# IntelRealSense/hand_tracking_samples

Hardware: AMD Instinct MI355X
Metric: synthetic depth frames/sec (CNN+solver), 64x64x1 input, 17-bone hand (higher is better)
Workload: dtype f32; 1 GPU; BASELINE configs[2]: 1024 independent 64x64 frames per GPU, CNN + decode + 5-step MultiStepSim + 3 FitPointCloud passes (GJK + PGS), 17 bones; frames_per_gpu=1024, parallelism=single GPU

## Files before the change

hand_tracking_samples_amd/csrc/ht_launch.hpp:

```cpp
#pragma once
#include "ht_device.hpp"

struct solve_args
{
	const float *rows_pre; const int *n_pre; int pre_stride;
	const float *rows_cloud; const int *n_cloud;
	const unsigned char *cloud_body;
	const float *contacts; const int *ncontacts;
	const float *ang_user; const int *n_ang_user; int ang_user_stride;
	const float *lin_tail; const int *n_lin_tail; int lin_tail_stride;
	const unsigned short *lin_tail_pos; const int *n_tail_groups;
	int no_model_rows;
	const float *analysis; const float *cams;
	const int *active_flag;
	float *state;
	float *scratch; int scratch_stride;
	int batch;
	int apply_angles; float drive_force; int ray_rows; int arm_cone; int zero_momenta; int steps_keyangles; float min_cray_prob;
	const float *sf_crays; int sf_ncray; int sf_select; float sf_spoint[3], sf_rbpoint[3]; const float *sf_refpose; int sf_hold;
	int *caps;
	int shared_gpu;
	const int *frame_order; int *cost_out;
	int two_body_levels;
	int force_build;
	float *out_poses; const int *out_npts; int *out_initializing; int out_min_point_num;
	int ang_extra_bound;
	float *exact_lin, *exact_ang;
	const float *tables;
	int dbg;
};

#define TB_WORDS 8928
struct prep_args
{
	const float *state; const float *analysis; const float *cams; const int *active_flag;
	float *scratch; int scratch_stride; int batch;
	const unsigned char *cloud_body; const int *n_cloud;
	const float *ch_planes; const int *ch_on;
	float *rows_pre; int *n_pre; float ch_maxforce;
	int apply_angles; float drive_force; int ray_rows; int arm_cone; int steps_keyangles; float min_cray_prob;
	int parts;
	float *tables;
	int dbg;
};
void ht_launch_solve_prep(const ht_model_dev &M, const ht_physics_dev &ph, const prep_args &a, int B, hipStream_t s);

struct cloud_records { float *scratch; int stride; unsigned char *body; float dt; };
void ht_launch_cloud_rows(const ht_model_dev &M, const float *state, const float4 *pts, const int *npts, const float *cams, const int *active_flag, int stride, int use_cam_origin, int mode,
                          const ht_params &par, float *rows, int *nrows, int B, hipStream_t s, float sf_ratio = 0.0f, float sf_wrist = 0.0f, const cloud_records *rec = nullptr);
struct ht_fit_after
{
	int mode;
	float reset_thr; int angles_only; int *flags, *nflags; int *list, *nlist; unsigned *nreset;
	float *hand; const float *other; const float *err_old; float *prev_err; int *initializing, *accepted; int nb, min_point_num, always_take_cnn; float accum_thr;
};
void ht_launch_fit_error(const ht_model_dev &M, const float *state, const float4 *pts, const int *npts, const uint16_t *depth, const float *cams, int w, int h, float scale, float *err, int B, hipStream_t s, const ht_fit_after *after = nullptr);
void ht_launch_chamber(const ht_model_dev &M, const float *state, const float4 *pts, const int *npts, int min_point_num, int enabled, float maxforce, float *rows, int *nch, int B, hipStream_t s,
                       const float *planes = nullptr, const int *planes_on = nullptr);
void ht_launch_chamber_planes(const ht_model_dev &M, const float4 *pts, const int *npts, int min_point_num, int enabled, float *planes, int *on, int B, hipStream_t s);
void ht_launch_contacts(const ht_model_dev &M, const float *state, float driftmax, float jiggle_sin, const int *active_flag, void *epa_ws, float *contacts, int *ncontacts, int B, hipStream_t s, bool beside_cloud_rows = false, int force_kernel = 0, int few_frames = 0,
                        const int *order = nullptr, int *work_out = nullptr);
int ht_contacts_frames_per_block(const ht_model_dev &M, int B);
#define HT_CONTACT_SLOTS 16
void ht_launch_order_by_points(const int *npts, int *order, int B, hipStream_t s);
void ht_launch_rank_desc(const int *work, int *order, int B, int stride, unsigned slots, int nslots, hipStream_t s);
void ht_launch_contact_order(const int *work, int *order, int B, int nfr, int stride, unsigned slots, int nslots, int epb, hipStream_t s);
size_t ht_contacts_workspace_bytes(int B);
void ht_launch_solve(const ht_model_dev &M, const ht_physics_dev &ph, const solve_args &a, int B, hipStream_t s);
void ht_launch_set_pose(float *state, const float *src, int nb, int n, int mode, hipStream_t s);
void ht_launch_get_state(const float *state, float *dst, int nb, int n, hipStream_t s);
void ht_launch_clear_flags(float *prev_err, int *initializing, int n, hipStream_t s);
void ht_launch_reset(const ht_model_dev &M, const ht_physics_dev &ph, float *state, const float4 *pts, const int *npts, const float *analysis, const float *cams, const int *list, const int *nlist,
                     int n_unibody, const ht_params &par, float *rows, int *nrows, float *scratch, int scratch_stride, int batch, int B, hipStream_t s, bool many_frames, int n_cu, bool exact = false);
void ht_launch_output(const ht_model_dev &M, const float *hand, const int *npts, int *initializing, int min_point_num, float *poses, int n, hipStream_t s, int raw = 0);
bool ht_segment_supported(int w, int h);
void ht_launch_segment(const uint16_t *depth, const float *cams, int w, int h, int entry_options, float wrange_hi, float diam, uint16_t *tiles, float *cams_out, int B, hipStream_t s);
void ht_launch_scale_state(float *state, int nb, int n, float s, hipStream_t st);
void ht_launch_train_step(float *w, float *W2p, const float *x, const float *target, float alpha, float *act, float *err, float *part, float *mse_out, hipStream_t s);
size_t ht_train_act_floats();
size_t ht_train_err_floats();
size_t ht_train_part_floats();
```

hand_tracking_samples_amd/csrc/ht_solver.hip:

```cpp
#include "ht_solve_shared.hpp"

template <int NGRP_, int NSUM_, int NANG_, int NIDX_, int AS_ = 2, int NCG_ = 0> struct lds_t
{
	static constexpr int NGRP = NGRP_, NSUM = NSUM_, NANG = NANG_, NIDX = NIDX_, MAXA2 = MAXA2_OF(AS_), NCG = NCG_;
	static constexpr int LIDLE = MAXG - 1;
	float pool[NGRP * LGRP] __attribute__((aligned(16)));
	float4 lin4[HT_MAXNB];
	float4 ang4[HT_MAXNB];
	float pos[HT_MAXNB][3], q[HT_MAXNB][4];
	float csum[NSUM];
	unsigned short cidx[NIDX > 0 ? NIDX : 2];
	float cg[NCG];
	int ccnt[HT_MAXNB], cstart[HT_MAXNB];
	signed char cextra[HT_MAXNB];
	union
	{
		unsigned lorder[MAXG];
		struct { unsigned short abody[128]; unsigned etmp[64]; } blk;
	};
	unsigned short lstart[MAXG + 2];
	unsigned aorder[MAXA2 + 1];
	unsigned short astart[MAXA2 + 2];
	int nlev_lin, nlev_ang, nray;
	union
	{
		struct
		{
			float jr[HT_MAXNJ][6];
			float ray[36][HT_ROW];
			int aprefix[HT_MAXNJ + 1], rprefix[HT_MAXNJ + 1];
			unsigned char rowj[MAXA2];
			unsigned char lrb[MAXG][2], arb[MAXA2][2];
			unsigned char gst[MAXA_RUNS + 1];
			float4 I4[HT_MAXNB][3];
		};
		float arec[(NANG + 4) * AROW] __attribute__((aligned(16)));
	};
};


template <int NS, class Order, class Start>
__device__ __forceinline__ int level_schedule(int n, int lane, const int (&b0)[2], const int (&b1)[2], Order put_order, Start put_start)
{
	auto rdl = [](int v, int l) -> int { return __builtin_amdgcn_readlane(v, l); };
	int last = 0, lev[2] = { 0, 0 };
	for (int g = 0; g < n; g++)
	{
		const int l = g & 63;
		const bool hi = NS > 1 && g >= 64;
		const int x0 = hi ? rdl(b0[1], l) : rdl(b0[0], l), x1 = hi ? rdl(b1[1], l) : rdl(b1[0], l);
		const int l0 = x0 != 255 ? rdl(last, x0 & 63) : 0, l1 = x1 != 255 ? rdl(last, x1 & 63) : 0;
		const int lv = (l0 > l1 ? l0 : l1) + 1;
		last = (lane == x0 || lane == x1) ? lv : last;
		lev[0] = (lane == l && !hi) ? lv : lev[0];
		if (NS > 1) lev[1] = (lane == l && hi) ? lv : lev[1];
	}
	int lower[2] = { 0, 0 }, before[2] = { 0, 0 };
	for (int h = 0; h < n; h++)
	{
		const int lh = (NS > 1 && h >= 64) ? rdl(lev[1], h & 63) : rdl(lev[0], h & 63);
#pragma unroll
		for (int s = 0; s < NS; s++) { lower[s] += lh < lev[s] ? 1 : 0; before[s] += (lh == lev[s] && h < lane + 64 * s) ? 1 : 0; }
	}
	int key[2], sb[2] = { 0, 0 };
#pragma unroll
	for (int s = 0; s < 2; s++) key[s] = (s < NS && lane + 64 * s < n) ? lev[s] * 2 + ((before[s] & 7) == 0 ? 1 : 0) : 0x7ffffffe;
	for (int h = 0; h < n; h++)
	{
		const int kh = (NS > 1 && h >= 64) ? rdl(key[1], h & 63) : rdl(key[0], h & 63);
#pragma unroll
		for (int s = 0; s < NS; s++) sb[s] += ((kh >> 1) < lev[s]) ? (kh & 1) : 0;
	}
	int steps = 0;
#pragma unroll
	for (int s = 0; s < NS; s++)
	{
		const int g = lane + 64 * s;
		const bool valid = g < n, first = valid && (before[s] & 7) == 0;
		const int pos = lower[s] + before[s];
		if (valid) put_order(pos, g, s);
		if (first) put_start(1 + sb[s] + (before[s] >> 3), pos);
		steps += __popcll(__ballot(first));
	}
	if (lane == 0) { put_start(steps + 1, n); put_start(steps + 2, n); }
	return steps;
}

#define EX_LIN HT_EX_LIN
template <int NGRP_, int NSUM_, int NANG_, int NIDX_, bool EXACT = false, int AS = 2, int NCG_ = 0>
__global__ __launch_bounds__(64, 2) void k_solve(ht_model_dev M, ht_physics_dev ph, solve_args a)
{
	__shared__ lds_t<NGRP_, NSUM_, NANG_, NIDX_, AS, NCG_> S;
	constexpr int ASLOTS = AS, MAXA2 = MAXA2_OF(AS), MAXA_LDS = MAXA_CAP_OF(AS);
	const int lane = threadIdx.x;
	const int b = a.frame_order ? a.frame_order[blockIdx.x] : (int)blockIdx.x;
	if (a.active_flag && !a.active_flag[b]) return;
	const long long t_cost = a.cost_out ? clock64() : 0;
	const long long t_entry = HT_DBG(a.dbg, 2048) ? clock64() : 0;
	const int nb = M.nb, nj = M.nj;
	float *st = a.state + (size_t)b * nb * HT_STATE_STRIDE;
	const float dt = ph.deltaT;
	const float *const T = a.tables ? a.tables + (size_t)b * TB_WORDS : nullptr;
	bool fast_pose = false, fast_chain = false;
	int t_na = 0, t_npre = 0, t_total = 0, t_e0 = 0, t_nblk = 0, t_head = 0;
	if constexpr (!EXACT)
	{
		if (T && !a.two_body_levels && !a.lin_tail && !a.ang_user && !a.no_model_rows && !(a.sf_refpose && a.sf_hold) && a.sf_select < 0 && a.sf_ncray == 0 && !a.rows_cloud)
		{
			const int h = lane < 32 ? reinterpret_cast<const int *>(T + TB_HDR)[lane] : 0;
			const int nc0 = (a.contacts && ph.use_collision) ? a.ncontacts[b] : 0;
			const int R = lane >> 4;
			t_na = __builtin_amdgcn_readlane(h, TH_NA); t_npre = __builtin_amdgcn_readlane(h, TH_NPRE); t_total = __builtin_amdgcn_readlane(h, TH_TOTAL);
			t_e0 = R == 0 ? __builtin_amdgcn_readlane(h, TH_E0) : R == 1 ? __builtin_amdgcn_readlane(h, TH_E0 + 1) : R == 2 ? __builtin_amdgcn_readlane(h, TH_E0 + 2) : __builtin_amdgcn_readlane(h, TH_E0 + 3);
			t_nblk = R == 0 ? __builtin_amdgcn_readlane(h, TH_NBLK) : R == 1 ? __builtin_amdgcn_readlane(h, TH_NBLK + 1) : R == 2 ? __builtin_amdgcn_readlane(h, TH_NBLK + 2) : __builtin_amdgcn_readlane(h, TH_NBLK + 3);
			t_head = R == 0 ? __builtin_amdgcn_readlane(h, TH_HEAD) : R == 1 ? __builtin_amdgcn_readlane(h, TH_HEAD + 1) : R == 2 ? __builtin_amdgcn_readlane(h, TH_HEAD + 2) : __builtin_amdgcn_readlane(h, TH_HEAD + 3);
			fast_pose = __builtin_amdgcn_readlane(h, TH_OK) != 0 && 3 * nj + 3 * (nc0 > HT_MAXCONTACT ? HT_MAXCONTACT : nc0) <= 4 * BLK_LROWS && !HT_DBG(a.dbg, 65536) && !HT_DBG(a.dbg, 1 << 22);
			fast_pose = __builtin_amdgcn_readfirstlane((int)fast_pose) != 0;
			fast_chain = fast_pose && __builtin_amdgcn_readlane(h, TH_CHAIN_OK) != 0;
			fast_chain = __builtin_amdgcn_readfirstlane((int)fast_chain) != 0;
		}
	}

	if (lane < nb)
	{
		const float *s = st + lane * HT_STATE_STRIDE;
		const float *bc = M.bodyc + lane * HT_BC;
		v3 lin = V3(s[7], s[8], s[9]), ang = V3(s[10], s[11], s[12]);
		const float damp = bc[HT_BC_DAMPLEFT];
		lin = lin * damp; ang = ang * damp;
		lin = lin + V3(0, 0, 0); ang = ang + V3(0, 0, 0);
		for (int i = 0; i < 3; i++) S.pos[lane][i] = s[i];
		for (int i = 0; i < 4; i++) S.q[lane][i] = s[3 + i];
		S.lin4[lane] = make_float4(lin.x, lin.y, lin.z, bc[HT_BC_MASSINV]);
		S.ang4[lane] = make_float4(ang.x, ang.y, ang.z, bc[HT_BC_FRICTION]);
		m3 I = world_inertia(V4(s[3], s[4], s[5], s[6]), LM(bc + HT_BC_TINV), bc[HT_BC_MASSINV]);
		S.I4[lane][0] = make_float4(I.x.x, I.x.y, I.x.z, 0.0f); S.I4[lane][1] = make_float4(I.y.x, I.y.y, I.y.z, 0.0f); S.I4[lane][2] = make_float4(I.z.x, I.z.y, I.z.z, 0.0f);
	}
	if (lane < nj && !fast_pose) for (int i = 0; i < 6; i++) S.jr[lane][i] = M.jointc[lane * HT_JC + HT_JC_RMIN + i];
	if (lane == 0) S.nray = fast_chain && a.ray_rows ? t_npre : 0;
	__syncthreads();

	if (nb >= 17 && !a.no_model_rows && !fast_pose)
	{
		if (lane < 4)
		{
			const int bb = 7 + 3 * lane;
			float c = clamp_std(dot(qzdir(L4(S.q[bb - 2])), qzdir(L4(S.q[bb - 1]))), 0.0f, 1.0f);
			float ang = (float)(acos((double)c) * (double)180.0f / (double)3.14159f / (double)2.0f);
			S.jr[bb - 1][3] = ang; S.jr[bb - 1][0] = ang;
		}
		else if (lane < 8)
		{
			const int k = lane - 4;
			const int kb = k == 0 ? 14 : k == 1 ? 11 : k == 2 ? 8 : 5;
			const float r0 = k == 0 ? -30.0f : -10.0f, r1 = k == 3 ? 20.0f : 10.0f;
			bool up = (double)dot(qydir(L4(S.q[1])), qydir(L4(S.q[kb]))) > ph.cos40d;
			S.jr[kb - 1][1] = up ? r0 : -0.0f;
			S.jr[kb - 1][4] = up ? r1 : 0.0f;
		}
	}
	if (fast_chain) {}
	else if (a.ray_rows && a.sf_ncray + (a.sf_select >= 0) > 0 && lane == 8)
	{
		int k = 0;
		for (int i = 0; i < a.sf_ncray && i < 8; i++)
		{
			const float *cr = a.sf_crays + ((size_t)b * 8 + i) * 4;
			v4 q = quat_from_to(V3(0, 0, 1), L3(cr));
			const int rb = FEATURE_BONE[i];
			const v3 off = V3(FEATURE_OFF[i][0], FEATURE_OFF[i][1], FEATURE_OFF[i][2]);
			for (int ax = 0; ax < 2; ax++)
			{
				const v3 axis = ax == 0 ? qxdir(q) : qydir(q);
				const float base = dot(anchor_world(S, rb, off) - V3(0, 0, 0), axis);
				for (int sd = 0; sd < 2; sd++)
				{
					float *o = S.ray[k++];
					o[0] = -1.0f; o[1] = (float)rb; o[2] = 0.0f; o[3] = 0.0f; o[4] = 0.0f; o[5] = off.x; o[6] = off.y; o[7] = off.z;
					o[8] = axis.x; o[9] = axis.y; o[10] = axis.z; o[11] = sd == 0 ? base + 0.01f : base - 0.01f; o[12] = 0.0f;
					o[13] = sd == 0 ? fmin_std(0.0f, 100000.0f) : fmin_std(-100000.0f, 0.0f); o[14] = sd == 0 ? fmax_std(0.0f, 100000.0f) : fmax_std(-100000.0f, 0.0f); o[15] = 0.0f;
				}
			}
		}
		if (a.sf_select >= 0)
		{
			const int rb = a.sf_select;
			const v3 sp = V3(a.sf_spoint[0], a.sf_spoint[1], a.sf_spoint[2]), rp = V3(a.sf_rbpoint[0], a.sf_rbpoint[1], a.sf_rbpoint[2]);
			const v3 d = anchor_world(S, rb, rp) - sp;
			for (int ax = 0; ax < 3; ax++)
			{
				float *o = S.ray[k++];
				o[0] = -1.0f; o[1] = (float)rb; o[2] = sp.x; o[3] = sp.y; o[4] = sp.z; o[5] = rp.x; o[6] = rp.y; o[7] = rp.z;
				o[8] = ax == 0 ? 1.0f : 0.0f; o[9] = ax == 1 ? 1.0f : 0.0f; o[10] = ax == 2 ? 1.0f : 0.0f; o[11] = ax == 0 ? d.x : ax == 1 ? d.y : d.z; o[12] = 0.0f;
				o[13] = -FLT_MAX; o[14] = FLT_MAX; o[15] = 0.0f;
			}
		}
		S.nray = k;
	}
	else if (a.ray_rows && lane == 8)
	{
		const float *an = a.analysis + (size_t)b * HT_ANALYSIS;
		const float *cam = a.cams + (size_t)b * HT_CAM;
		const v3 campos = V3(cam[5], cam[6], cam[7]);
		int k = 0;
		for (int i = (a.steps_keyangles ? 3 : 0); i < 8; i++)
			if (i >= 3 && an[HT_AN_CLENCH + i - 3] < 3.14f / 2.0f && an[HT_AN_CRAYS + 4 * i + 3] >= a.min_cray_prob)
			{
				v4 q = quat_from_to(V3(0, 0, 1), L3(an + HT_AN_CRAYS + 4 * i));
				const int rb = FEATURE_BONE[i];
				const v3 off = V3(FEATURE_OFF[i][0], FEATURE_OFF[i][1], FEATURE_OFF[i][2]);
				for (int ax = 0; ax < 2; ax++)
				{
					const v3 axis = ax == 0 ? qxdir(q) : qydir(q);
					const float base = dot(anchor_world(S, rb, off) - campos, axis);
					for (int side = 0; side < 2; side++)
					{
						float *o = S.ray[k++];
						o[0] = -1.0f; o[1] = (float)rb; o[2] = campos.x; o[3] = campos.y; o[4] = campos.z; o[5] = off.x; o[6] = off.y; o[7] = off.z;
						o[8] = axis.x; o[9] = axis.y; o[10] = axis.z; o[11] = side == 0 ? base + 0.01f : base - 0.01f; o[12] = 0.0f;
						o[13] = side == 0 ? fmin_std(0.0f, 100000.0f) : fmin_std(-100000.0f, 0.0f); o[14] = side == 0 ? fmax_std(0.0f, 100000.0f) : fmax_std(-100000.0f, 0.0f); o[15] = 0.0f;
					}
				}
			}
		S.nray = k;
	}
	__syncthreads();
	if (HT_DBG(a.dbg, 256)) return;
	const long long t_m1 = HT_DBG(a.dbg, 2048) ? clock64() : 0;
	const bool rel = a.sf_refpose && a.sf_hold;
	const int na_user = a.ang_user ? (a.n_ang_user[b] < MAXA_LDS ? a.n_ang_user[b] : MAXA_LDS) : 0;
	int na_pre, na;
	const int na_fix = na_user + (a.apply_angles ? 12 : 0) + (a.arm_cone ? 1 : 0);
	if (fast_pose) { na_pre = na_fix; na = t_na; }
	else
	{
		const int acnt = (lane < nj && !a.no_model_rows) ? angular_range_count(L3(S.jr[lane]), L3(S.jr[lane] + 3)) : 0;
		int rcnt = 0;
		if (rel && lane < nj && ((lane != 0 && a.sf_hold == 2) || lane > 3)) for (int ax = 0; ax < 3; ax++) rcnt += S.jr[lane][ax] != S.jr[lane][3 + ax];
		int rpre = 0, apre = 0, rtot = 0, atot = 0;
		for (int j = 0; j < nj; j++)
		{
			const int rc = __builtin_amdgcn_readlane(rcnt, j), ac = __builtin_amdgcn_readlane(acnt, j);
			rpre += j < lane ? rc : 0; apre += j < lane ? ac : 0; rtot += rc; atot += ac;
		}
		na_pre = na_fix + rtot; na = na_pre + atot;
		if (lane <= nj) { S.rprefix[lane] = na_fix + rpre; S.aprefix[lane] = na_pre + apre; }
		for (int k = 0; k < acnt; k++) if (na_pre + apre + k < MAXA2) S.rowj[na_pre + apre + k] = (unsigned char)lane;
	}
	__syncthreads();
	if (na > MAXA_LDS && a.caps && lane == 0) atomicAdd(a.caps, 1);
	if (na > MAXA2) na = MAXA2;
	arow AR[ASLOTS];
#pragma unroll
	for (int s = 0; s < ASLOTS; s++)
	{
		const int r = lane + 64 * s;
		arow &R = AR[s];
		R.rb0 = -1; R.rb1 = -1; R.axis = V3(0, 0, 1); R.targetspin = -FLT_MAX; R.mn = 0; R.mx = 0; R.s2t = 0; R.torque = 0; R.mintorque = 0; R.lev = 0;
		if (r < na && !fast_pose)
		{
			float row[8];
			if (r < na_user)
			{
				const float *u = a.ang_user + ((size_t)b * a.ang_user_stride + r) * HT_AROW;
				put_ang(row, (int)u[0], (int)u[1], V3(u[2], u[3], u[4]), u[5], u[6], u[7]);
			}
			else if (r < na_fix)
			{
				const float *cam = a.cams + (size_t)b * HT_CAM;
				const v4 camq = V4(cam[8], cam[9], cam[10], cam[11]);
				const int ra = a.apply_angles ? r - na_user : 12;
				if (ra == 12) cone_angle(ph, S, -1, qrot(camq, V3(0, -1, 0)), 0, V3(0, 0, 1), 70.0f, row);
				else
				{
					const float *an = a.analysis + (size_t)b * HT_ANALYSIS;
					const float *fc = an + HT_AN_CLENCH;
					if (ra < 3)
					{
						float tmp[3][8];
						angular_drive(ph, S, -1, 1, qmul(camq, V4(an[HT_AN_PALMQ], an[HT_AN_PALMQ + 1], an[HT_AN_PALMQ + 2], an[HT_AN_PALMQ + 3])), a.drive_force, tmp);
						for (int k = 0; k < 8; k++) row[k] = ra == 0 ? tmp[0][k] : ra == 1 ? tmp[1][k] : tmp[2][k];
					}
					else if (ra == 3) { float th = fc[0]; cone_angle(ph, S, 1, V3((float)cos((double)th), 0, (float)sin((double)th)), 4, V3(0, 0, 1), 10.0f, row); }
					else
					{
						const int finger = 1 + (ra - 4) / 2;
						const float aa = fc[finger];
						if (((ra - 4) & 1) == 0) cone_angle(ph, S, 1, V3(0, (float)(-sin((double)aa)), (float)cos((double)aa)), 3 + finger * 3, V3(0, 0, 1), 10.0f, row);
						else
						{
							v4 jf = L4(M.jointc + (1 + finger * 3) * HT_JC + HT_JC_FRAME);
							v3 inner = V3(0, (float)(-sin((double)(aa / 2.0f))), (float)cos((double)(aa / 2.0f)));
							cone_angle(ph, S, 1, qrot(jf, qrot(jf, inner)), 2 + finger * 3, V3(0, 0, 1), 10.0f, row);
						}
					}
				}
			}
			else if (r < na_pre)
			{
				int j = 0;
				while (j + 1 < nj && S.rprefix[j + 1] <= r) j++;
				int sub = r - S.rprefix[j], ax = 0;
				for (int k = 0; k < 3; k++) if (S.jr[j][k] != S.jr[j][3 + k]) { if (sub == 0) { ax = k; sub = -1; } else if (sub > 0) sub--; }
				const float *jc = M.jointc + j * HT_JC;
				const int rb0 = (int)jc[HT_JC_RB0], rb1 = (int)jc[HT_JC_RB1];
				const float *r0 = a.sf_refpose + ((size_t)b * nb + rb0) * HT_POSE, *r1 = a.sf_refpose + ((size_t)b * nb + rb1) * HT_POSE;
				const xf ref0 = XF(L3(r0), L4(r0 + 3)), ref1 = XF(L3(r1), L4(r1 + 3));
				const xf dq = mul(mul(inverse(mul(inverse(ref0), ref1)), inverse(body_xf(S, rb0))), body_xf(S, rb1));
				const m3 R0 = qmat(L4(S.q[rb0]));
				const v3 axis = ax == 0 ? R0.x : ax == 1 ? R0.y : R0.z;
				const float qa = ax == 0 ? dq.q.x : ax == 1 ? dq.q.y : dq.q.z;
				put_ang(row, rb0, rb1, axis, -qa * 2.0f / dt, -FLT_MAX, FLT_MAX);
			}
			else
			{
				const int j = S.rowj[r];
				const int sub = r - S.aprefix[j];
				const float *jc = M.jointc + j * HT_JC;
				const int rb0 = (int)jc[HT_JC_RB0], rb1 = (int)jc[HT_JC_RB1];
				const v4 jf = L4(jc + HT_JC_FRAME);
				angular_range_row(ph, rb0, rb0 >= 0 ? qmul(L4(S.q[rb0]), jf) : jf, rb1, rb1 >= 0 ? L4(S.q[rb1]) : V4(0, 0, 0, 1), L3(S.jr[j]), L3(S.jr[j] + 3), sub, row);
			}
			R.rb0 = __float_as_int(row[0]); R.rb1 = __float_as_int(row[1]); R.axis = V3(row[2], row[3], row[4]); R.targetspin = row[5];
			const float mintorque = row[6], maxtorque = row[7];
			R.s2t = 1.0f / (((R.rb0 >= 0) ? dot(R.axis, mul(body_I(S, R.rb0), R.axis)) : 0.0f) + ((R.rb1 >= 0) ? dot(R.axis, mul(body_I(S, R.rb1), R.axis)) : 0.0f));
			R.mn = mintorque * dt; R.mx = maxtorque * dt; R.mintorque = mintorque; R.torque = 0.0f;
			if constexpr (EXACT) { float *e = a.exact_ang + ((size_t)b * 256 + r) * 8; for (int k = 0; k < 8; k++) e[k] = row[k]; }
			S.arb[r][0] = (unsigned char)(R.rb0 >= 0 ? R.rb0 : 255); S.arb[r][1] = (unsigned char)(R.rb1 >= 0 ? R.rb1 : 255);
		}
	}

	if (HT_DBG(a.dbg, 512)) return;
	const long long t_m2 = HT_DBG(a.dbg, 2048) ? clock64() : 0;
	int nc = (a.contacts && ph.use_collision) ? a.ncontacts[b] : 0;
	if (nc > HT_MAXCONTACT) nc = HT_MAXCONTACT;
	const int njg = a.no_model_rows ? 0 : nj;
	const int nt = a.lin_tail ? a.n_lin_tail[b] : 0, ngt = a.lin_tail ? a.n_tail_groups[b] : 0;
	const int n2 = nt + 3 * njg + 3 * nc, ng2 = ngt + njg + nc;
	const bool seq_lin = ng2 > MAXG - 1;
	const int rec_cap = a.scratch_stride - HT_SCRATCH_TAIL;
	float *scr = a.scratch + (size_t)b * a.scratch_stride * CREC;
	const bool pool_lds = ng2 + 1 <= S.NGRP;
	float *const gpool = scr + (size_t)rec_cap * CREC, *const garec = gpool + MAXG_CAP * LGRP;
	float *const pool = pool_lds ? S.pool : gpool;
	if (ngt > 0)
	{
		for (int i = lane; i < ngt * LGRP; i += 64) pool[i] = ((i % LGRP) >= LG_RINV && (i % LGRP) < LG_RINV + 3) ? 1.0f : 0.0f;
		__threadfence_block();
		__syncthreads();
	}
	if (fast_pose)
	{
		const float4 *src = reinterpret_cast<const float4 *>(T + TB_POOL);
		for (int i = lane; i < njg * (LGRP / 4); i += 64) reinterpret_cast<float4 *>(pool)[i] = src[i];
	}
	for (int r = (fast_pose ? 3 * njg : 0) + lane; r < n2; r += 64)
	{
		int rb0, rb1, meta = 0, g, kk;
		v3 p0, p1, n; float targetdist, tsnb, fmn, fmx;
		if (r < nt)
		{
			const float *u = a.lin_tail + ((size_t)b * a.lin_tail_stride + r) * HT_ROW;
			const unsigned pos = a.lin_tail_pos[(size_t)b * a.lin_tail_stride + r];
			g = (int)((pos & 0x7FFF) >> 2); kk = (int)(pos & 3);
			rb0 = (int)u[0]; rb1 = (int)u[1]; p0 = L3(u + 2); p1 = L3(u + 5); n = L3(u + 8); targetdist = u[11]; tsnb = u[12]; fmn = u[13]; fmx = u[14];
			if (pos & 0x8000) meta = kk == 0 ? LM_NORMAL : LM_FRIC;
		}
		else if (r < nt + 3 * njg)
		{
			const int j = (r - nt) / 3, ax = (r - nt) % 3;
			g = ngt + j; kk = ax;
			const float *jc = M.jointc + j * HT_JC;
			rb0 = (int)jc[HT_JC_RB0]; rb1 = (int)jc[HT_JC_RB1];
			p0 = L3(jc + HT_JC_P0) - L3(M.bodyc + rb0 * HT_BC + HT_BC_COM); p1 = L3(jc + HT_JC_P1) - L3(M.bodyc + rb1 * HT_BC + HT_BC_COM);
			const v3 d = anchor_world(S, rb1, p1) - anchor_world(S, rb0, p0);
			n = V3(ax == 0 ? 1.0f : 0.0f, ax == 1 ? 1.0f : 0.0f, ax == 2 ? 1.0f : 0.0f);
			targetdist = ax == 0 ? d.x : ax == 1 ? d.y : d.z; tsnb = 0.0f; fmn = -FLT_MAX; fmx = FLT_MAX;
		}
		else
		{
			const int ci = (r - nt - 3 * njg) / 3, k = (r - nt - 3 * njg) % 3;
			g = ngt + njg + ci; kk = k;
			const float *c = a.contacts + ((size_t)b * HT_MAXCONTACT + ci) * HT_CONTACT;
			rb0 = (int)c[0]; rb1 = (int)c[1];
			const v3 normal = L3(c + 2), p0w = L3(c + 5), p1w = L3(c + 8);
			const float separation = c[11];
			p0 = apply(inverse(body_xf(S, rb0)), p0w); p1 = apply(inverse(body_xf(S, rb1)), p1w);
			if (k == 0)
			{
				const v3 r0w = p0w - L3(S.pos[rb0]), r1w = p1w - L3(S.pos[rb1]);
				const v3 v0 = cross(spin_of(S, rb0), r0w) + F3(S.lin4[rb0]) * S.lin4[rb0].w;
				const v3 v1 = cross(spin_of(S, rb1), r1w) + F3(S.lin4[rb1]) * S.lin4[rb1].w;
				const v3 v = v0 - v1;
				const float minsep = ph.driftmax * 0.25f;
				const float bouncevel = fmax_std(0.0f, (-dot(normal, v) - ph.gravity_len * ph.falltime_to_ballistic) * ph.restitution);
				n = -normal; targetdist = fmin_std((separation - minsep) * ph.biasfactorpositive, separation); tsnb = -bouncevel; fmn = 0; fmx = FLT_MAX;
				meta = LM_NORMAL;
			}
			else
			{
				v4 q = quat_from_to(V3(0, 0, 1), -normal);
				n = k == 1 ? qydir(q) : qxdir(q);
				targetdist = 0; tsnb = 0; fmn = 0;
				fmx = 0;
				meta = LM_FRIC;
			}
		}
		if constexpr (EXACT)
		{
			if (r < EX_LIN)
			{
				float *e = a.exact_lin + ((size_t)b * EX_LIN + r) * HT_ROW;
				e[0] = (float)rb0; e[1] = (float)rb1; e[2] = p0.x; e[3] = p0.y; e[4] = p0.z; e[5] = p1.x; e[6] = p1.y; e[7] = p1.z; e[8] = n.x; e[9] = n.y; e[10] = n.z;
				e[11] = targetdist; e[12] = tsnb; e[13] = fmin_std(fmn, fmx); e[14] = fmax_std(fmn, fmx); e[15] = (meta & LM_FRIC) ? (float)-kk : 0.0f;
			}
		}
		const m3 Z = { V3(0, 0, 0), V3(0, 0, 0), V3(0, 0, 0) };
		const v3 r0 = rb0 >= 0 ? qrot(L4(S.q[rb0]), p0) : p0, r1 = rb1 >= 0 ? qrot(L4(S.q[rb1]), p1) : p1;
		const m3 I0 = rb0 >= 0 ? body_I(S, rb0) : Z, I1 = rb1 >= 0 ? body_I(S, rb1) : Z;
		const float impulsed = (rb0 >= 0 ? S.lin4[rb0].w + dot(cross(mul(I0, cross(r0, n)), r0), n) : 0.0f) + (rb1 >= 0 ? S.lin4[rb1].w + dot(cross(mul(I1, cross(r1, n)), r1), n) : 0.0f);
		const float ts = targetdist / dt;
		const v3 g0 = -cross(r0, n), g1 = cross(r1, n), b0 = mul(I0, g0), b1 = mul(I1, g1);
		float *o = pool + g * LGRP;
		float *os = o + LG_S + 4 * kk;
		os[0] = ts; os[1] = fmin_std(ts, tsnb); os[2] = fmin_std(fmn, fmx) * dt; os[3] = fmax_std(fmn, fmx) * dt;
		if (meta & LM_FRIC) os[3] = fmax_std(rb0 >= 0 ? S.ang4[rb0].w : 0.0f, rb1 >= 0 ? S.ang4[rb1].w : 0.0f);
		o[LG_RINV + kk] = 1.0f / impulsed; o[LG_SUM + kk] = 0.0f;
		if (kk == 0) o[LG_META] = __int_as_float(meta | (rb0 & 255) | ((rb1 & 255) << 8));
		o[LG_N + 3 * kk] = n.x; o[LG_N + 3 * kk + 1] = n.y; o[LG_N + 3 * kk + 2] = n.z;
		float *og = o + LG_GB + 12 * kk;
		og[0] = g0.x; og[1] = b0.x; og[2] = g0.y; og[3] = b0.y; og[4] = g0.z; og[5] = b0.z;
		og[6] = g1.x; og[7] = b1.x; og[8] = g1.y; og[9] = b1.y; og[10] = g1.z; og[11] = b1.z;
		if (kk == 0 && g < MAXG) { S.lrb[g][0] = (unsigned char)(rb0 >= 0 ? rb0 : 255); S.lrb[g][1] = (unsigned char)(rb1 >= 0 ? rb1 : 255); }
	}
	if (lane < LGRP) pool[ng2 * LGRP + lane] = (lane >= LG_RINV && lane < LG_RINV + 3) ? 1.0f : lane == LG_META ? __int_as_float(IDLE_BODY | (IDLE_BODY << 8)) : 0.0f;
	if (lane == 0)
	{
		S.lin4[IDLE_BODY] = make_float4(0, 0, 0, 0); S.ang4[IDLE_BODY] = make_float4(0, 0, 0, 0);
		S.I4[IDLE_BODY][0] = S.I4[IDLE_BODY][1] = S.I4[IDLE_BODY][2] = make_float4(0, 0, 0, 0);
		S.lorder[S.LIDLE] = (unsigned)ng2 | ((unsigned)IDLE_BODY << 16) | ((unsigned)IDLE_BODY << 24);
	}
	__threadfence_block();
	__syncthreads();
	const long long t_m2b = HT_DBG(a.dbg, 2048) ? clock64() : 0;
	if (na > MAXA_LDS) na = MAXA_LDS;
	bool blocked = false;
	if constexpr (!EXACT)
	{
		bool sw = false;
#pragma unroll
		for (int s = 0; s < ASLOTS; s++) sw = sw || (lane + 64 * s < na && AR[s].targetspin == -FLT_MAX && AR[s].mintorque < 0);
		blocked = !a.two_body_levels && ngt == 0 && n2 <= 4 * BLK_LROWS && na <= 128 && __ballot(sw) == 0ull;
		blocked = __builtin_amdgcn_readfirstlane((int)blocked) != 0;
		if (fast_pose) blocked = true;
	}
	int nga = 0;
	if (!blocked)
	for (int base = 0; base < na; base += 64)
	{
		const int r = base + lane;
		const bool head = r < na && (r == 0 || S.arb[r][0] != S.arb[r - 1][0] || S.arb[r][1] != S.arb[r - 1][1]);
		const unsigned long long m = __ballot(head);
		const int k = nga + __popcll(m & ((1ull << lane) - 1ull));
		if (head && k <= MAXA_RUNS) S.gst[k] = (unsigned char)r;
		nga += __popcll(m);
	}
	__syncthreads();
	if (nga > MAXA_RUNS)
	{
		if (a.caps && lane == 0) atomicAdd(a.caps, 1);
		na = S.gst[MAXA_RUNS]; nga = MAXA_RUNS;
	}
	if (blocked) { if (lane == 0) { S.nlev_lin = 0; S.nlev_ang = 0; } }
	else
	{
		int gb0[2], gb1[2];
		const int ngs = seq_lin ? 0 : ng2;
#pragma unroll
		for (int s = 0; s < 2; s++) { const int g = lane + 64 * s; gb0[s] = g < ngs ? S.lrb[g][0] : 255; gb1[s] = g < ngs ? S.lrb[g][1] : 255; }
		auto put_lorder = [&](int pos, int g, int s) { S.lorder[pos] = (unsigned)g | ((unsigned)(gb0[s] == 255 ? IDLE_BODY : gb0[s]) << 16) | ((unsigned)(gb1[s] == 255 ? IDLE_BODY : gb1[s]) << 24); };
		auto put_lstart = [&](int step, int v) { S.lstart[step] = (unsigned short)v; };
		int nl = ngs <= 64 ? level_schedule<1>(ngs, lane, gb0, gb1, put_lorder, put_lstart) : level_schedule<2>(ngs, lane, gb0, gb1, put_lorder, put_lstart);
		if (seq_lin) nl = ng2;
		int ar[2], ac[2];
#pragma unroll
		for (int s = 0; s < 2; s++)
		{
			const int g = lane + 64 * s;
			ar[s] = g < nga ? (int)S.gst[g] : 0;
			ac[s] = (g + 1 < nga ? (int)S.gst[g + 1] : na) - ar[s];
			gb0[s] = g < nga ? S.arb[ar[s]][0] : 255; gb1[s] = g < nga ? S.arb[ar[s]][1] : 255;
		}
		auto put_aorder = [&](int pos, int g, int s) { S.aorder[pos] = (unsigned)ar[s] | ((unsigned)ac[s] << 8) | ((unsigned)(gb0[s] == 255 ? IDLE_BODY : gb0[s]) << 16) | ((unsigned)(gb1[s] == 255 ? IDLE_BODY : gb1[s]) << 24); };
		auto put_astart = [&](int step, int v) { S.astart[step] = (unsigned short)v; };
		const int nla = nga <= 64 ? level_schedule<1>(nga, lane, gb0, gb1, put_aorder, put_astart) : level_schedule<2>(nga, lane, gb0, gb1, put_aorder, put_astart);
		if (lane == 0)
		{
			S.nlev_lin = nl; S.nlev_ang = nla;
			S.aorder[MAXA2] = (unsigned)na | (1u << 8) | ((unsigned)IDLE_BODY << 16) | ((unsigned)IDLE_BODY << 24);
		}
	}
	__syncthreads();
	const int nlev_lin = S.nlev_lin, nlev_ang = S.nlev_ang;
	if (HT_DBG(a.dbg, 64)) return;
	const long long t_m3 = HT_DBG(a.dbg, 2048) ? clock64() : 0;

	const int npre_g = a.rows_pre ? a.n_pre[b] : 0;
	const int npre = a.ray_rows ? S.nray : npre_g;
	const int ncl = (a.rows_cloud || a.cloud_body) ? a.n_cloud[b] : 0;
	const int n1 = npre + ncl;
	const int pre_base = M.pts_cap, noop_idx = rec_cap - 1;
	const int npad_max = 7 * (nb > 16 ? nb - 16 : 0);
	const int nlist = n1 + (npad_max > 3 * nb ? npad_max : 3 * nb) + (QUAD_CHAIN_SLACK > QUAD_BLOCK_SLACK ? QUAD_CHAIN_SLACK : QUAD_BLOCK_SLACK);
	const bool sums_lds = nlist <= S.NSUM;
	const bool idx_lds = sums_lds && nlist <= S.NIDX && rec_cap <= 65536;
	float *const gsum = a.scratch + (size_t)a.batch * a.scratch_stride * CREC + (size_t)b * a.scratch_stride;
	unsigned *const gidx = reinterpret_cast<unsigned *>(a.scratch + (size_t)a.batch * a.scratch_stride * (CREC + 1)) + (size_t)b * a.scratch_stride;
	float *const gG = a.scratch + (size_t)a.batch * a.scratch_stride * (CREC + 2) + (size_t)b * a.scratch_stride * 4;
	if (sums_lds) { for (int i = lane; i < nlist; i += 64) S.csum[i] = 0.0f; }
	else for (int i = lane; i < nlist && i < a.scratch_stride; i += 64) gsum[i] = 0.0f;
	if (fast_chain) { if (idx_lds) for (int i = lane; i < nlist; i += 64) S.cidx[i] = (unsigned short)gidx[i]; }
	else if (idx_lds) { for (int i = lane; i < nlist; i += 64) S.cidx[i] = (unsigned short)noop_idx; }
	else for (int i = lane; i < nlist && i < a.scratch_stride; i += 64) gidx[i] = (unsigned)noop_idx;
	if (lane == 0 && !fast_chain) quad_write_noop(scr + (size_t)noop_idx * CREC);
	auto pre_ptr = [&](int i) -> const float * { return a.ray_rows ? S.ray[i] : a.rows_pre + ((size_t)b * a.pre_stride + i) * HT_ROW; };
	auto body_of = [&](int i) -> int {
		if (i < npre) return (int)pre_ptr(i)[1];
		if (a.cloud_body) return (int)a.cloud_body[(size_t)b * M.pts_cap + (i - npre)];
		return (int)a.rows_cloud[((size_t)b * M.pts_cap + (i - npre)) * HT_ROW + 1];
	};
	__syncthreads();
	int mycnt = 0;
	if (!fast_chain)
	for (int base = 0; base < n1; base += 64)
	{
		const int i = base + lane;
		int body = (i < n1) ? body_of(i) : -1;
		unsigned long long todo = __ballot(body >= 0);
		while (todo)
		{
			const int leader = __ffsll((long long)todo) - 1;
			const int bb = __builtin_amdgcn_readlane(body, leader);
			const unsigned long long m = __ballot(body == bb);
			if (lane == bb) mycnt += __popcll(m);
			todo &= ~m;
		}
	}
	const long long t_l1 = HT_DBG(a.dbg, 262144) ? clock64() : 0;
	const bool chain4 = !EXACT && !HT_DBG(a.dbg, 65536);
	int c4_e0 = 0, c4_nblk = 0, c4_head = 0, c4_start = 0, c4_next = -1, c4_total = 0;
	int myblk = (lane < nb && !HT_DBG(a.dbg, 1)) ? (mycnt + 3) >> 2 : 0;
	if (fast_chain)
	{
		c4_e0 = t_e0; c4_nblk = t_nblk; c4_head = t_head; c4_total = t_total;
		if (lane < HT_MAXNB) { myblk = reinterpret_cast<const int *>(T + TB_CCNT)[lane]; c4_next = reinterpret_cast<const int *>(T + TB_CNEXT)[lane]; }
	}
	else if (chain4)
	{
		int myrank = 0;
		for (int k = 0; k < nb; k++) { const int o = __builtin_amdgcn_readlane(myblk, k); myrank += (o > myblk || (o == myblk && k < lane)) ? 1 : 0; }
		if (lane < nb) S.cstart[myrank] = lane;
		__builtin_amdgcn_fence(__ATOMIC_SEQ_CST, "wavefront");
		__builtin_amdgcn_wave_barrier();
		const int sorted = lane < nb ? S.cstart[lane] : 0;
		int ld0 = 0, ld1 = 0, ld2 = 0, ld3 = 0, la0 = -1, la1 = -1, la2 = -1, la3 = -1, hd0 = 0, hd1 = 0, hd2 = 0, hd3 = 0, myrow = 0, mypos = 0;
		for (int r = 0; r < nb; r++)
		{
			const int bb = __builtin_amdgcn_readlane(sorted, r);
			const int blk = __builtin_amdgcn_readlane(myblk, bb);
			if (blk == 0) break;
			int row = 0, best = ld0;
			if (ld1 < best) { row = 1; best = ld1; }
			if (ld2 < best) { row = 2; best = ld2; }
			if (ld3 < best) { row = 3; best = ld3; }
			const int prev = row == 0 ? la0 : row == 1 ? la1 : row == 2 ? la2 : la3;
			if (lane == bb) { myrow = row; mypos = best; }
			if (lane == prev) c4_next = bb;
			if (prev < 0) { if (row == 0) hd0 = bb; else if (row == 1) hd1 = bb; else if (row == 2) hd2 = bb; else hd3 = bb; }
			if (row == 0) { la0 = bb; ld0 += blk; } else if (row == 1) { la1 = bb; ld1 += blk; } else if (row == 2) { la2 = bb; ld2 += blk; } else { la3 = bb; ld3 += blk; }
		}
		const int sg1 = 4 * ld0, sg2 = sg1 + 4 * ld1, sg3 = sg2 + 4 * ld2;
		c4_total = ld0 + ld1 + ld2 + ld3;
		c4_start = (myrow == 0 ? 0 : myrow == 1 ? sg1 : myrow == 2 ? sg2 : sg3) + 4 * mypos;
		const int R = lane >> 4;
		c4_e0 = R == 0 ? 0 : R == 1 ? sg1 : R == 2 ? sg2 : sg3; c4_nblk = R == 0 ? ld0 : R == 1 ? ld1 : R == 2 ? ld2 : ld3; c4_head = R == 0 ? hd0 : R == 1 ? hd1 : R == 2 ? hd2 : hd3;
	}
	int myextra = -1, myhost = -1;
	if (!fast_chain)
	{
		int avail = (lane < 16 && lane < nb) ? mycnt : 0x7fffff;
		for (int e = 16; e < nb; e++)
		{
			int key = (avail << 6) | lane;
#pragma unroll
			for (int o = 1; o < 64; o <<= 1) { const int v = __shfl_xor(key, o); key = v < key ? v : key; }
			const int h = key & 63;
			if (lane == h) { myextra = e; avail = 0x7fffff; }
			if (lane == e) myhost = h;
		}
	}
	const int extracnt = __shfl(mycnt, myextra >= 0 ? myextra : lane);
	const int mylen = lane >= 16 ? 0 : (myextra >= 0 && extracnt > 0 ? ((mycnt + 7) & ~7) + extracnt : mycnt);
	if (myextra >= 0 && extracnt == 0) myextra = -1;
	int mystart = mylen;
#pragma unroll
	for (int o = 1; o < 64; o <<= 1) { int v = __shfl_up(mystart, o); if (lane >= o) mystart += v; }
	mystart -= mylen;
	{
		const int hs = __shfl(mystart, myhost >= 0 ? myhost : lane), hc = __shfl(mycnt, myhost >= 0 ? myhost : lane);
		if (myhost >= 0) mystart = hs + ((hc + 7) & ~7);
	}
	if (chain4) { mystart = c4_start; if (lane < HT_MAXNB) { S.ccnt[lane] = myblk; S.cstart[lane] = mystart; S.cextra[lane] = (signed char)c4_next; } }
	else if (lane < HT_MAXNB) { S.ccnt[lane] = HT_DBG(a.dbg, 1) ? 0 : mycnt; S.cstart[lane] = mystart; S.cextra[lane] = (signed char)(HT_DBG(a.dbg, 1) ? -1 : myextra); }
	int myrun = 0;
	const long long t_l2 = HT_DBG(a.dbg, 262144) ? clock64() : 0;
	if (!fast_chain)
	for (int base = 0; base < n1; base += 64)
	{
		const int i = base + lane;
		int body = (i < n1) ? body_of(i) : -1;
		int dst = -1;
		unsigned long long todo = __ballot(body >= 0);
		while (todo)
		{
			const int leader = __ffsll((long long)todo) - 1;
			const int bb = __builtin_amdgcn_readlane(body, leader);
			const unsigned long long m = __ballot(body == bb);
			const int segbase = __builtin_amdgcn_readlane(mystart + myrun, bb);
			if (body == bb) dst = segbase + __popcll(m & ((1ull << lane) - 1ull));
			if (lane == bb) myrun += __popcll(m);
			todo &= ~m;
		}
		if (body >= 0)
		{
			const bool made = i >= npre && a.cloud_body;
			const int src = i < npre ? pre_base + i : i - npre;
			if (src < noop_idx && dst < nlist - QUAD_CHAIN_SLACK)
			{
				if (idx_lds) S.cidx[dst] = (unsigned short)src; else if (dst < a.scratch_stride) gidx[dst] = (unsigned)src;
				if (!made)
				{
					const float *r = i < npre ? pre_ptr(i) : a.rows_cloud + ((size_t)b * M.pts_cap + (i - npre)) * HT_ROW;
					const v3 p1 = L3(r + 5), n = L3(r + 8);
					const v3 r1 = qrot(L4(S.q[body]), p1);
					const m3 Ib = body_I(S, body);
					const float impulsed = S.lin4[body].w + dot(cross(mul(Ib, cross(r1, n)), r1), n);
					const float ts = r[11] / dt;
					quad_write_record(scr + (size_t)src * CREC, r1, n, Ib, S.lin4[body].w, ts, fmin_std(ts, r[12]), impulsed, r[13] * dt, r[14] * dt);
				}
			}
		}
	}
	const long long t_l3 = HT_DBG(a.dbg, 262144) ? clock64() : 0;
	v3 ABA0[ASLOTS], ABA1[ASLOTS];
#pragma unroll
	for (int s = 0; s < ASLOTS; s++)
	{
		const arow &R = AR[s];
		const bool on = lane + 64 * s < na && !fast_pose;
		ABA0[s] = (on && R.rb0 >= 0) ? -mul(body_I(S, R.rb0), R.axis) : V3(0, 0, 0);
		ABA1[s] = (on && R.rb1 >= 0) ? mul(body_I(S, R.rb1), R.axis) : V3(0, 0, 0);
	}
	__threadfence_block();
	__syncthreads();
	const bool g_lds = idx_lds && S.NCG > 0 && QUAD_G_BLOCK * (c4_total + 4) <= S.NCG;
	if (fast_chain)
	{
		if (g_lds) { for (int i = lane; i < QUAD_G_BLOCK * c4_total; i += 64) S.cg[i] = gG[i]; __threadfence_block(); __syncthreads(); }
	}
	else if (chain4 && !HT_DBG(a.dbg, 131072))
	{
		const int quad_ = lane >> 2, c_ = lane & 3;
		for (int blk0 = quad_; blk0 < c4_total; blk0 += 64)
		{
			float4 r_[4][4];
#pragma unroll
			for (int u = 0; u < 4; u++)
#pragma unroll
				for (int j = 0; j < 4; j++)
				{
					const int blk = blk0 + 16 * u, e = 4 * blk + j;
					const unsigned x = (blk < c4_total) ? (idx_lds ? (unsigned)S.cidx[e] : gidx[e]) : (unsigned)noop_idx;
					r_[u][j] = reinterpret_cast<const float4 *>(scr + (size_t)x * CREC)[c_];
				}
#pragma unroll
			for (int u = 0; u < 4; u++)
			{
				const int blk = blk0 + 16 * u;
				auto coup = [&](int j, int i) -> float {
					const float p = __fmaf_rn(r_[u][j].z, r_[u][i].y, r_[u][j].x * r_[u][i].w);
					const float t = dpp<QP_PREV>(p) + p;
					return -(dpp<QP_PREV>(t) + p);
				};
				const float g10 = coup(1, 0), g20 = coup(2, 0), g21 = coup(2, 1), g30 = coup(3, 0), g31 = coup(3, 1), g32 = coup(3, 2);
				if (c_ == 2 && blk < c4_total && 4 * blk + 3 < a.scratch_stride)
				{
					float2 *o = reinterpret_cast<float2 *>((g_lds ? S.cg : gG) + QUAD_G_BLOCK * blk);
					o[0] = make_float2(g30, g31); o[1] = make_float2(g32, g20); o[2] = make_float2(g21, 0.0f); o[3] = make_float2(g10, 0.0f); o[4] = make_float2(0.0f, 0.0f);
				}
			}
		}
		__threadfence_block();
		__syncthreads();
	}
	const long long t_l4 = HT_DBG(a.dbg, 262144) ? clock64() : 0;
	v3 pos_next = V3(0, 0, 0); v4 q_next = V4(0, 0, 0, 1);
	auto calc_next_pose = [&]() {
		const float *bc = M.bodyc + lane * HT_BC;
		const float minv = S.lin4[lane].w;
		pos_next = L3(S.pos[lane]) + (F3(S.lin4[lane]) * minv) * dt;
		const m3 tinv = LM(bc + HT_BC_TINV) * minv;
		const v3 angm = F3(S.ang4[lane]);
		const v4 s = L4(S.q[lane]);
		auto diffq = [&](v4 o) -> v4 {
			v4 sn = normalize(o);
			m3 Mx = qmat(sn);
			m3 Ii = mul(Mx, mul(tinv, transpose(Mx)));
			v3 hs = mul(Ii, angm) * 0.5f;
			return qmul(V4(hs.x, hs.y, hs.z, 0), sn);
		};
		v4 d1 = diffq(s), d2 = diffq(s + d1 * (dt / 2)), d3 = diffq(s + d2 * (dt / 2)), d4 = diffq(s + d3 * dt);
		v4 o = normalize((((s + d1 * (dt / 6)) + d2 * (dt / 3)) + d3 * (dt / 3)) + d4 * (dt / 6));
		if (o.x < FLT_EPSILON / 4.0f && o.x > -FLT_EPSILON / 4.0f) o.x = 0.0f;
		if (o.y < FLT_EPSILON / 4.0f && o.y > -FLT_EPSILON / 4.0f) o.y = 0.0f;
		if (o.z < FLT_EPSILON / 4.0f && o.z > -FLT_EPSILON / 4.0f) o.z = 0.0f;
		q_next = o;
	};
	if constexpr (EXACT)
	{
		const int nlin2 = n2 < EX_LIN ? n2 : EX_LIN;
		float *const sums = gsum;
		for (int i = lane; i < n1 + nlin2 + na && i < a.scratch_stride; i += 64) sums[i] = 0.0f;
		__threadfence_block();
		__syncthreads();
		auto sweeps = [&](int count, bool post) {
			auto linear = [&](int rb0, int rb1, v3 p0, v3 p1, v3 n, float ts, float fx, float fy, float *sum) {
				const m3 Z = { V3(0, 0, 0), V3(0, 0, 0), V3(0, 0, 0) };
				const v3 r0 = rb0 >= 0 ? qrot(L4(S.q[rb0]), p0) : p0, r1 = rb1 >= 0 ? qrot(L4(S.q[rb1]), p1) : p1;
				const v3 v0 = rb0 >= 0 ? cross(spin_of(S, rb0), r0) + F3(S.lin4[rb0]) * S.lin4[rb0].w : V3(0, 0, 0);
				const v3 v1 = rb1 >= 0 ? cross(spin_of(S, rb1), r1) + F3(S.lin4[rb1]) * S.lin4[rb1].w : V3(0, 0, 0);
				const float vn = dot(v1 - v0, n);
				const float impulsen = -ts - vn;
				const float impulsed = (rb0 >= 0 ? S.lin4[rb0].w + dot(cross(mul(body_I(S, rb0), cross(r0, n)), r0), n) : 0.0f)
				                     + (rb1 >= 0 ? S.lin4[rb1].w + dot(cross(mul(body_I(S, rb1), cross(r1, n)), r1), n) : 0.0f);
				float impulse = impulsen / impulsed;
				const float isum = *sum;
				impulse = fmin_std(fy * dt - isum, impulse);
				impulse = fmax_std(fx * dt - isum, impulse);
				if (rb0 >= 0)
				{
					const v3 im = n * -impulse;
					const v3 l = F3(S.lin4[rb0]) + im, av = F3(S.ang4[rb0]) + cross(r0, im);
					S.lin4[rb0].x = l.x; S.lin4[rb0].y = l.y; S.lin4[rb0].z = l.z; S.ang4[rb0].x = av.x; S.ang4[rb0].y = av.y; S.ang4[rb0].z = av.z;
				}
				if (rb1 >= 0)
				{
					const v3 im = n * impulse;
					const v3 l = F3(S.lin4[rb1]) + im, av = F3(S.ang4[rb1]) + cross(r1, im);
					S.lin4[rb1].x = l.x; S.lin4[rb1].y = l.y; S.lin4[rb1].z = l.z; S.ang4[rb1].x = av.x; S.ang4[rb1].y = av.y; S.ang4[rb1].z = av.z;
				}
				*sum = isum + impulse;
				(void)Z;
			};
			for (int sw = 0; sw < count; sw++)
			{
				for (int i = 0; i < n1; i++)
				{
					const float *r = i < npre ? pre_ptr(i) : a.rows_cloud + ((size_t)b * M.pts_cap + (i - npre)) * HT_ROW;
					const float ts = r[11] / dt;
					linear((int)r[0], (int)r[1], L3(r + 2), L3(r + 5), L3(r + 8), post ? fmin_std(ts, r[12]) : ts, r[13], r[14], sums + i);
				}
				for (int i = 0; i < nlin2; i++)
				{
					const float *r = a.exact_lin + ((size_t)b * EX_LIN + i) * HT_ROW;
					const int rb0 = (int)r[0], rb1 = (int)r[1], fm = (int)r[15];
					const float ts = r[11] / dt;
					float fx = r[13], fy = r[14];
					if (fm)
					{
						fy = fmax_std(rb0 >= 0 ? S.ang4[rb0].w : 0.0f, rb1 >= 0 ? S.ang4[rb1].w : 0.0f) * sums[n1 + i + fm] / dt;
						fx = -fy;
					}
					linear(rb0, rb1, L3(r + 2), L3(r + 5), L3(r + 8), post ? fmin_std(ts, r[12]) : ts, fx, fy, sums + n1 + i);
				}
				for (int i = 0; i < na; i++)
				{
					const float *r = a.exact_ang + ((size_t)b * 256 + i) * 8;
					const int rb0 = __float_as_int(r[0]), rb1 = __float_as_int(r[1]);
					const v3 axis = L3(r + 2);
					const float mintorque = r[6], maxtorque = r[7];
					const float targetspin = post ? ((mintorque < 0) ? 0 : fmin_std(r[5], 0.0f)) : r[5];
					if (targetspin == -FLT_MAX) continue;
					const float currentspin = ((rb1 >= 0) ? dot(spin_of(S, rb1), axis) : 0.0f) - ((rb0 >= 0) ? dot(spin_of(S, rb0), axis) : 0.0f);
					const float dspin = targetspin - currentspin;
					const float spintotorque = 1.0f / (((rb0 >= 0) ? dot(axis, mul(body_I(S, rb0), axis)) : 0.0f) + ((rb1 >= 0) ? dot(axis, mul(body_I(S, rb1), axis)) : 0.0f));
					float dtorque = dspin * spintotorque;
					float *tq = sums + n1 + nlin2 + i;
					const float torque = *tq;
					dtorque = fmin_std(dtorque, maxtorque * dt - torque);
					dtorque = fmax_std(dtorque, mintorque * dt - torque);
					if (rb0 >= 0) { const v3 av = F3(S.ang4[rb0]) - axis * dtorque; S.ang4[rb0].x = av.x; S.ang4[rb0].y = av.y; S.ang4[rb0].z = av.z; }
					if (rb1 >= 0) { const v3 av = F3(S.ang4[rb1]) + axis * dtorque; S.ang4[rb1].x = av.x; S.ang4[rb1].y = av.y; S.ang4[rb1].z = av.z; }
					*tq = torque + dtorque;
				}
			}
		};
		if (lane == 0) sweeps(ph.iterations, false);
		__threadfence_block();
		__syncthreads();
		if (lane < nb) calc_next_pose();
		__syncthreads();
		if (lane == 0) sweeps(ph.iterations_post, true);
		__threadfence_block();
		__syncthreads();
	}
	else
	{
	const bool arec_lds = na <= S.NANG;
	float *const arec = arec_lds ? S.arec : garec;
	if (fast_pose)
	{
		const float4 *src = reinterpret_cast<const float4 *>(T + TB_AREC);
		for (int i = lane; i < (na + 4) * (AROW / 4); i += 64) reinterpret_cast<float4 *>(arec)[i] = src[i];
		const unsigned w = reinterpret_cast<const unsigned *>(T + TB_ABODY)[lane];
		S.blk.abody[2 * lane] = (unsigned short)(w & 0xFFFFu); S.blk.abody[2 * lane + 1] = (unsigned short)(w >> 16);
	}
	else
	{
#pragma unroll
	for (int s = 0; s < ASLOTS; s++)
	{
		const int r = lane + 64 * s;
		if (r < na)
		{
			const arow &R = AR[s];
			float *o = arec + r * AROW;
			const float ts_post = (R.mintorque < 0) ? 0 : fmin_std(R.targetspin, 0.0f);
			o[AR_S] = R.targetspin; o[AR_S + 1] = ts_post; o[AR_S + 2] = R.mn; o[AR_S + 3] = R.mx;
			o[AR_GAIN] = R.targetspin == -FLT_MAX ? 0.0f : R.s2t; o[AR_TORQUE] = 0.0f;
			o[AR_AXIS] = R.axis.x; o[AR_AXIS + 1] = R.axis.y; o[AR_AXIS + 2] = R.axis.z; o[AR_AXIS + 3] = ts_post == -FLT_MAX ? 0.0f : R.s2t;
			const v3 ba0 = ABA0[s], ba1 = ABA1[s];
			o[AR_BA] = ba0.x; o[AR_BA + 1] = ba0.y; o[AR_BA + 2] = ba0.z; o[AR_BA + 3] = ba1.x; o[AR_BA + 4] = ba1.y; o[AR_BA + 5] = ba1.z;
		}
	}
	if (lane < 4 * AROW) arec[na * AROW + lane] = 0.0f;
	if (blocked)
	{
#pragma unroll
		for (int s = 0; s < 2; s++)
		{
			const int r = lane + 64 * s;
			S.blk.abody[r] = (unsigned short)(r < na ? ((AR[s].rb0 >= 0 ? AR[s].rb0 : 255) | ((AR[s].rb1 >= 0 ? AR[s].rb1 : 255) << 8)) : 0xFFFF);
		}
	}
	}
	__threadfence_block();
	__syncthreads();

	float GL[32], GA[32];
	unsigned emL0 = 0, emL1 = 0, emL2 = 0, emL3 = 0, emA0 = 0, emA1 = 0, emA2 = 0, emA3 = 0;
	unsigned lbod = 0xFFFFFFFFu, abod = 0xFFFFFFFFu;
#pragma unroll
	for (int i = 0; i < 32; i++) { GL[i] = 0.0f; GA[i] = 0.0f; }
	const int nbl = blocked ? (n2 + BLK_LROWS - 1) / BLK_LROWS : 0, nba = blocked ? (na + 31) >> 5 : 0;
	long long t_c0 = 0, t_c1 = 0, t_c2 = 0;
	if (blocked)
	{
		if (HT_DBG(a.dbg, 2048)) t_c0 = clock64();
		const int m = lane & 31, hh = lane >> 5;
		{
			auto lbodies = [&](int Q) -> unsigned {
				const int p = (Q & 1) ? 31 - m : m, row = BLK_LROWS * Q + p;
				const bool on = p < BLK_LROWS && row < n2;
				return on ? ((unsigned)__float_as_int(pool[(row / 3) * LGRP + LG_META]) & 0xFFFFu) : 0xFFFFu;
			};
			auto abodies = [&](int Q) -> unsigned { const int row = 32 * Q + ((Q & 1) ? 31 - m : m); return row < na ? (unsigned)S.blk.abody[row] : 0xFFFFu; };
			lbod = lbodies(2 * hh) | (lbodies(2 * hh + 1) << 16);
			abod = abodies(2 * hh) | (abodies(2 * hh + 1) << 16);
		}
		auto ang_couplings = [&](const auto arec_, const bool bwd) {
			const int r = bwd ? 64 * hh + 63 - m : 64 * hh + m;
			const float *R = arec_ + (r < na ? r : na) * AROW;
			const float ng = -R[AR_GAIN];
			const v3 b0 = L3(R + AR_BA) * ng, b1 = L3(R + AR_BA + 3) * ng;
			const int bo = (int)S.blk.abody[r], a0 = bo & 255, a1 = bo >> 8;
#pragma unroll
			for (int c8 = 0; c8 < 32; c8 += 8)
			{
				float ax[8], ay[8], az[8]; int pb[8];
#pragma unroll
				for (int u = 0; u < 8; u++)
				{
					const int rp = bwd ? 64 * hh + 63 - (c8 + u) : 64 * hh + c8 + u;
					const float *P = arec_ + (rp < na ? rp : na) * AROW + AR_AXIS;
					ax[u] = P[0]; ay[u] = P[1]; az[u] = P[2]; pb[u] = (int)S.blk.abody[rp];
				}
#pragma unroll
				for (int u = 0; u < 8; u++)
				{
					const int rho = c8 + u, p0 = pb[u] & 255, p1 = pb[u] >> 8;
					const float t0 = (b0.x * ax[u] + b0.y * ay[u]) + b0.z * az[u], t1 = (b1.x * ax[u] + b1.y * ay[u]) + b1.z * az[u];
					float g = (a0 == p1 ? t0 : a0 == p0 ? -t0 : 0.0f) + (a1 == p1 ? t1 : a1 == p0 ? -t1 : 0.0f);
					asm volatile("" : "+v"(g));
					GA[rho] = (bwd ? rho > m : rho < m) ? g : GA[rho];
				}
			}
		};
		if (fast_pose)
		{
#pragma unroll
			for (int k = 0; k < 8; k++)
			{
				const float4 ga = reinterpret_cast<const float4 *>(T + TB_GA)[k * 64 + lane], gl = reinterpret_cast<const float4 *>(T + TB_GL)[k * 64 + lane];
				GA[4 * k] = ga.x; GA[4 * k + 1] = ga.y; GA[4 * k + 2] = ga.z; GA[4 * k + 3] = ga.w;
				GL[4 * k] = gl.x; GL[4 * k + 1] = gl.y; GL[4 * k + 2] = gl.z; GL[4 * k + 3] = gl.w;
			}
		}
		else if (arec_lds) { ang_couplings(S.arec, false); if (nba > 1) ang_couplings(S.arec, true); }
		else { ang_couplings(garec, false); if (nba > 1) ang_couplings(garec, true); }
		auto lin_couplings = [&](const auto pool_, const bool bwd) {
			const int blk = 2 * hh + (bwd ? 1 : 0), pos = bwd ? 31 - m : m, row = BLK_LROWS * blk + pos;
			const bool on = pos < BLK_LROWS && row < n2;
			const int g_ = on ? row / 3 : ng2, k_ = on ? row - 3 * g_ : 0;
			const float *R = pool_ + g_ * LGRP;
			const float nr = on ? -R[LG_RINV + k_] : 0.0f;
			const v3 n = L3(R + LG_N + 3 * k_) * nr;
			const float *og = R + LG_GB + 12 * k_;
			const v3 b0 = V3(og[1], og[3], og[5]) * nr, b1 = V3(og[7], og[9], og[11]) * nr;
			const unsigned bo = bwd ? lbod >> 16 : lbod & 0xFFFFu;
			const int a0 = (int)(bo & 255u), a1 = (int)(bo >> 8);
			const float ma = S.lin4[a0 < HT_MAXNB ? a0 : IDLE_BODY].w, mb = S.lin4[a1 < HT_MAXNB ? a1 : IDLE_BODY].w;
#pragma unroll
			for (int c4 = 0; c4 < 32; c4 += 4)
			{
				float pn[4][3], q0[4][3], q1[4][3]; int pb[4];
#pragma unroll
				for (int u = 0; u < 4; u++)
				{
					const int ppos = bwd ? 31 - (c4 + u) : c4 + u, prow = BLK_LROWS * blk + ppos;
					const bool pon = ppos >= 0 && ppos < BLK_LROWS && prow < n2;
					const int pg = pon ? 10 * blk + ppos / 3 : ng2, pk = pon ? ppos % 3 : 0;
					const float *P = pool_ + pg * LGRP;
					const float *pgb = P + LG_GB + 12 * pk;
					pn[u][0] = P[LG_N + 3 * pk]; pn[u][1] = P[LG_N + 3 * pk + 1]; pn[u][2] = P[LG_N + 3 * pk + 2];
					q0[u][0] = pgb[0]; q0[u][1] = pgb[2]; q0[u][2] = pgb[4]; q1[u][0] = pgb[6]; q1[u][1] = pgb[8]; q1[u][2] = pgb[10];
					pb[u] = __float_as_int(P[LG_META]);
				}
#pragma unroll
				for (int u = 0; u < 4; u++)
				{
					const int rho = c4 + u, p0 = pb[u] & 255, p1 = (pb[u] >> 8) & 255;
					const bool daa = a0 == p0, dab = a0 == p1, dba = a1 == p0, dbb = a1 == p1;
					const float t00 = (b0.x * q0[u][0] + b0.y * q0[u][1]) + b0.z * q0[u][2], t01 = (b0.x * q1[u][0] + b0.y * q1[u][1]) + b0.z * q1[u][2];
					const float t10 = (b1.x * q0[u][0] + b1.y * q0[u][1]) + b1.z * q0[u][2], t11 = (b1.x * q1[u][0] + b1.y * q1[u][1]) + b1.z * q1[u][2];
					const float nn = (n.x * pn[u][0] + n.y * pn[u][1]) + n.z * pn[u][2];
					const float mm = (daa ? ma : dab ? -ma : 0.0f) + (dbb ? mb : dba ? -mb : 0.0f);
					float g = ((daa ? t00 : dab ? t01 : 0.0f) + (dba ? t10 : dbb ? t11 : 0.0f)) + nn * mm;
					asm volatile("" : "+v"(g));
					GL[rho] = (bwd ? rho > m : rho < m) ? g : GL[rho];
				}
			}
		};
		const int njr = 3 * njg;
		auto has_contacts = [&](int Q) -> bool { return n2 > njr && BLK_LROWS * Q < n2 && BLK_LROWS * (Q + 1) > njr; };
		const bool fwd = !fast_pose || has_contacts(0) || has_contacts(2), bwd = !fast_pose || has_contacts(1) || has_contacts(3);
		if (pool_lds) { if (nbl > 0 && fwd) lin_couplings(S.pool, false); if (nbl > 1 && bwd) lin_couplings(S.pool, true); }
		else { if (nbl > 0 && fwd) lin_couplings(gpool, false); if (nbl > 1 && bwd) lin_couplings(gpool, true); }
		if (HT_DBG(a.dbg, 2048)) t_c1 = clock64();
		auto edge_word = [&](bool valid, int ba, int bb) -> unsigned {
			const int ka = (valid && ba < nb) ? ba : 255, kb = (valid && bb < nb) ? bb : 255;
			const unsigned long long lt = (1ull << lane) - 1ull;
			int r0 = -1, r1 = -1, base = 0;
			unsigned pm = (ka < 32 ? 1u << ka : 0u) | (kb < 32 ? 1u << kb : 0u);
			pm |= (unsigned)__builtin_amdgcn_update_dpp(0, (int)pm, 0x111, 0xF, 0xF, false); pm |= (unsigned)__builtin_amdgcn_update_dpp(0, (int)pm, 0x112, 0xF, 0xF, false);
			pm |= (unsigned)__builtin_amdgcn_update_dpp(0, (int)pm, 0x114, 0xF, 0xF, false); pm |= (unsigned)__builtin_amdgcn_update_dpp(0, (int)pm, 0x118, 0xF, 0xF, false);
			pm |= (unsigned)__builtin_amdgcn_update_dpp(0, (int)pm, 0x142, 0xA, 0xF, false); pm |= (unsigned)__builtin_amdgcn_update_dpp(0, (int)pm, 0x143, 0xC, 0xF, false);
			pm = (unsigned)__builtin_amdgcn_readlane((int)pm, 63);
			while (pm)
			{
				const int k = __ffs((int)pm) - 1;
				pm &= pm - 1u;
				const unsigned long long m0 = __ballot(ka == k), m1 = __ballot(kb == k);
				const int below = __popcll((m0 | m1) & lt);
				if (ka == k) r0 = base + below;
				if (kb == k) r1 = base + below;
				base += __popcll(m0) + __popcll(m1);
			}
			__syncthreads();
			S.blk.etmp[lane] = 0u;
			__threadfence_block();
			__syncthreads();
			if (r0 >= 0) S.blk.etmp[r0] = (unsigned)lane | BLK_E_VALID | ((unsigned)ka << 16);
			if (r1 >= 0) S.blk.etmp[r1] = (unsigned)lane | BLK_E_SIDE | BLK_E_VALID | ((unsigned)kb << 16);
			__threadfence_block();
			__syncthreads();
			const unsigned e = S.blk.etmp[lane];
			const bool v = (e & BLK_E_VALID) != 0;
			auto same = [&](int other) -> bool { const unsigned o = S.blk.etmp[other & 63]; return v && other >= 0 && other < 64 && (o & BLK_E_VALID) != 0 && (o >> 16) == (e >> 16); };
			const int rs = lane & ~15;
			unsigned w = e;
			if (v && !same(lane + 1)) w |= BLK_E_TAIL;
			if (lane - 1 >= rs && same(lane - 1)) w |= 1u << 9;
			if (lane - 2 >= rs && same(lane - 2)) w |= 1u << 10;
			if (lane - 4 >= rs && same(lane - 4)) w |= 1u << 11;
			if (lane - 8 >= rs && same(lane - 8)) w |= 1u << 12;
			if ((lane & 16) && same(rs - 1)) w |= 1u << 13;
			if (lane >= 32 && same(31)) w |= 1u << 14;
			return w;
// ... 115 lines not shown
			__builtin_amdgcn_wave_barrier();
			momenta(Bs, l, av);
			__builtin_amdgcn_sched_barrier(0);
			fetch(A, e_a); e_b = entry(L + 3);
			__builtin_amdgcn_sched_barrier(0);
			step(Bs, l, av);
			__builtin_amdgcn_wave_barrier();
		}
	};
	auto angular_phase = [&](const auto arec_, const auto post_c) {
		constexpr bool POST = decltype(post_c)::value;
		struct aset { unsigned e; float ax, ba, ts, mn, mx, gain, torque; };
		auto entry = [&](int L) -> unsigned {
			if (L > nlev_ang) return S.aorder[MAXA2];
			int lo, hi;
			if (L < 63) { lo = __builtin_amdgcn_readlane(ls_ang, L); hi = __builtin_amdgcn_readlane(ls_ang, L + 1); }
			else { lo = S.astart[L]; hi = S.astart[L + 1]; }
			const int idx = lo + pslot;
			return S.aorder[idx < hi ? idx : MAXA2];
		};
		auto load = [&](aset &r, const float *R) {
			const float4 sv = *reinterpret_cast<const float4 *>(R + AR_S); const float2 gt = *reinterpret_cast<const float2 *>(R + AR_GAIN);
			r.ts = POST ? sv.y : sv.x; r.mn = sv.z; r.mx = sv.w; r.gain = POST ? R[AR_AXIS + 3] : gt.x; r.torque = gt.y;
			r.ax = R[AR_AXIS + cc]; r.ba = R[AR_BA + 3 * side + cc];
		};
		auto fetch = [&](aset &r, unsigned e) { r.e = e; load(r, arec_ + (int)(e & 0xFF) * AROW); };
		auto momentum = [&](const aset &r) -> float { const int body = side ? (int)(r.e >> 24) : (int)((r.e >> 16) & 255); return ang_w[4 * body + c]; };
		auto apply = [&](const aset &r, float *R, float &av) {
			const float axs = __int_as_float(__float_as_int(r.ax) ^ sidesign);
			const float gain = r.gain;
			const float p = r.ba * av;
			const float sp = (dpp<QP_BC0>(p) + dpp<QP_BC1>(p)) + dpp<QP_BC2>(p);
			const float currentspin = sp + pair_other_uniform(sp);
			float dtorque = (r.ts - currentspin) * gain;
			dtorque = clamp_med3(dtorque, r.mn - r.torque, r.mx - r.torque);
			av = __fmaf_rn(axs, dtorque, av);
			R[AR_TORQUE] = r.torque + dtorque;
		};
		auto step = [&](const aset &r0, float av) {
			const int body = side ? (int)(r0.e >> 24) : (int)((r0.e >> 16) & 255);
			const int cnt = HT_DBG(a.dbg, 16384) ? 1 : (int)((r0.e >> 8) & 255);
			const bool bv = body != IDLE_BODY;
			float *R = arec_ + (int)(r0.e & 0xFF) * AROW;
			aset ra = r0, rb, rc;
			load(rb, R + AROW);
			for (int k = 0;;)
			{
				load(rc, R + 2 * AROW); apply(ra, R, av); if (++k >= cnt) break;
				load(ra, R + 3 * AROW); apply(rb, R + AROW, av); if (++k >= cnt) break;
				load(rb, R + 4 * AROW); apply(rc, R + 2 * AROW, av); if (++k >= cnt) break;
				R += 3 * AROW;
			}
			if (c < 3 && bv) ang_w[4 * body + c] = av;
		};
		aset A, Bs;
		fetch(A, entry(1));
		unsigned e_b = entry(2), e_a;
		for (int L = 1; L <= nlev_ang; L += 2)
		{
			float av = momentum(A);
			__builtin_amdgcn_sched_barrier(0);
			fetch(Bs, e_b); e_a = entry(L + 2);
			__builtin_amdgcn_sched_barrier(0);
			step(A, av);
			if (L + 1 > nlev_ang) break;
			__builtin_amdgcn_wave_barrier();
			av = momentum(Bs);
			__builtin_amdgcn_sched_barrier(0);
			fetch(A, e_a); e_b = entry(L + 3);
			__builtin_amdgcn_sched_barrier(0);
			step(Bs, av);
			__builtin_amdgcn_wave_barrier();
		}
	};
	const int idt_bits = __builtin_amdgcn_readfirstlane(__float_as_int(inv_dt)), dt_bits = __builtin_amdgcn_readfirstlane(__float_as_int(dt));
	auto blocked_linear = [&](const auto pool_, const bool post) {
		for (int Q = 0; Q < nbl; Q++)
		{
			const long long tb0 = stats ? clock64() : 0;
			const int m = lane & 31;
			const int p = (Q & 1) ? 31 - m : m, row = BLK_LROWS * Q + p;
			const bool act = (lane >> 5) == (Q >> 1) && p < BLK_LROWS && row < n2;
			const int g = act ? row / 3 : ng2, k = act ? row - 3 * g : 0;
			auto *const R = pool_ + g * LGRP;
			const float4 sv = *reinterpret_cast<const float4 *>(R + LG_S + 4 * k);
			const float rinv = R[LG_RINV + k], sum = R[LG_SUM + k], fms = R[LG_SUM];
			const v3 n = L3(R + LG_N + 3 * k);
			const float4 o0 = *reinterpret_cast<const float4 *>(R + LG_GB + 12 * k), o1 = *reinterpret_cast<const float4 *>(R + LG_GB + 12 * k + 4), o2 = *reinterpret_cast<const float4 *>(R + LG_GB + 12 * k + 8);
			const v3 g0 = V3(o0.x, o0.z, o1.x), b0 = V3(o0.y, o0.w, o1.y), g1 = V3(o1.z, o2.x, o2.z), b1 = V3(o1.w, o2.y, o2.w);
			const unsigned bo = act ? ((Q & 1) ? lbod >> 16 : lbod & 0xFFFFu) : 0xFFFFu;
			const int ba = (bo & 255u) < HT_MAXNB ? (int)(bo & 255u) : IDLE_BODY, bb = (bo >> 8) < HT_MAXNB ? (int)(bo >> 8) : IDLE_BODY;
			const bool contact = g >= njg && g < ng2;
			const float4 Pa = S.lin4[ba], La = S.ang4[ba], Pb = S.lin4[bb], Lb = S.ang4[bb];
			float w = b0.x * La.x; w = __fmaf_rn(b0.y, La.y, w); w = __fmaf_rn(b0.z, La.z, w);
			w = __fmaf_rn(b1.x, Lb.x, w); w = __fmaf_rn(b1.y, Lb.y, w); w = __fmaf_rn(b1.z, Lb.z, w);
			const float na_ = -Pa.w, nb_ = Pb.w;
			w = __fmaf_rn(n.x * na_, Pa.x, w); w = __fmaf_rn(n.y * na_, Pa.y, w); w = __fmaf_rn(n.z * na_, Pa.z, w);
			w = __fmaf_rn(n.x * nb_, Pb.x, w); w = __fmaf_rn(n.y * nb_, Pb.y, w); w = __fmaf_rn(n.z * nb_, Pb.z, w);
			float x = (-(post ? sv.y : sv.x) - w) * rinv;
			const bool fric = act && k > 0 && contact;
			float lo = fric ? 0.0f : sv.z - sum, hi = fric ? 0.0f : sv.w - sum;
			const int mp = fric ? p - k : 255;
			float imp = 0.0f;
			const int nrows = n2 - BLK_LROWS * Q;
			long long tb1 = 0; if (stats) { asm volatile("" :: "v"(x), "v"(lo), "v"(hi)); tb1 = clock64(); }
			int cwl[2]; bool gen[2];
#pragma unroll
			for (int hf = 0; hf < 2; hf++)
			{
				const int g0_ = 10 * Q + 5 * hf;
				int np = ng2 - g0_, fc = njg - g0_;
				np = np < 0 ? 0 : np > 5 ? 5 : np; fc = fc < 0 ? 0 : fc > 5 ? 5 : fc;
				const int pres = (1 << np) - 1;
				cwl[hf] = __builtin_amdgcn_readfirstlane((pres << 8) | (pres & ~((1 << fc) - 1)));
				gen[hf] = __builtin_amdgcn_readfirstlane((int)(fc < 5 || np < 5)) != 0;
			}
#define BLK_LHALF(QQ, HF) if (gen[HF]) blk_resolve15<QQ, HF, true>(x, lo, hi, imp, GL, fms, sv.w, sum, mp, idt_bits, dt_bits, cwl[HF]); else blk_resolve15<QQ, HF, false>(x, lo, hi, imp, GL, fms, sv.w, sum, mp, idt_bits, dt_bits, 0);
#define BLK_LCASE(QQ) case QQ: BLK_LHALF(QQ, 0) if (nrows > 15) { BLK_LHALF(QQ, 1) } break;
			switch (Q) { BLK_LCASE(0) BLK_LCASE(1) BLK_LCASE(2) default: BLK_LCASE(3) }
#undef BLK_LHALF
#undef BLK_LCASE
			long long tb2 = 0; if (stats) { asm volatile("" :: "v"(imp)); tb2 = clock64(); }
			if (act) R[LG_SUM + k] = sum + imp;
			const unsigned e = Q == 0 ? emL0 : Q == 1 ? emL1 : Q == 2 ? emL2 : emL3;
			const int src = (int)(e & 63);
			const bool side = (e & BLK_E_SIDE) != 0;
			const float cf = (e & BLK_E_VALID) ? (side ? 1.0f : -1.0f) : 0.0f, cv = (e & BLK_E_VALID) ? 1.0f : 0.0f;
			const float dpx = n.x * imp, dpy = n.y * imp, dpz = n.z * imp;
			const float d0x = g0.x * imp, d0y = g0.y * imp, d0z = g0.z * imp, d1x = g1.x * imp, d1y = g1.y * imp, d1z = g1.z * imp;
			float vpx = blk_pull(src, dpx) * cf, vpy = blk_pull(src, dpy) * cf, vpz = blk_pull(src, dpz) * cf;
			const float q0x = blk_pull(src, d0x), q0y = blk_pull(src, d0y), q0z = blk_pull(src, d0z), q1x = blk_pull(src, d1x), q1y = blk_pull(src, d1y), q1z = blk_pull(src, d1z);
			float vlx = (side ? q1x : q0x) * cv, vly = (side ? q1y : q0y) * cv, vlz = (side ? q1z : q0z) * cv;
			const blk_scan_mul sm = blk_scan_multipliers(e);
			blk_seg_scan3(vpx, vpy, vpz, sm);
			blk_seg_scan3(vlx, vly, vlz, sm);
			if (e & BLK_E_TAIL)
			{
				const int body = (int)(e >> 16);
				float4 P = S.lin4[body], L = S.ang4[body];
				P.x += vpx; P.y += vpy; P.z += vpz; L.x += vlx; L.y += vly; L.z += vlz;
				S.lin4[body] = P; S.ang4[body] = L;
			}
			__builtin_amdgcn_wave_barrier();
			if (stats) { asm volatile("s_waitcnt lgkmcnt(0)" ::: "memory"); const long long tb3 = clock64(); cyc_bh += tb1 - tb0; cyc_br += tb2 - tb1; cyc_bg += tb3 - tb2; }
		}
	};
	auto blocked_angular = [&](const auto arec_, const bool post) {
		for (int Q = 0; Q < nba; Q++)
		{
			const int m = lane & 31;
			const int p = (Q & 1) ? 31 - m : m, row = 32 * Q + p;
			const bool act = (lane >> 5) == (Q >> 1) && row < na;
			auto *const R = arec_ + (act ? row : na) * AROW;
			const float4 sv = *reinterpret_cast<const float4 *>(R + AR_S), gt = *reinterpret_cast<const float4 *>(R + AR_GAIN), ab = *reinterpret_cast<const float4 *>(R + AR_AXIS + 2), bt = *reinterpret_cast<const float4 *>(R + AR_BA + 2);
			const unsigned bo = act ? ((Q & 1) ? abod >> 16 : abod & 0xFFFFu) : 0xFFFFu;
			const int ba = (bo & 255u) < HT_MAXNB ? (int)(bo & 255u) : IDLE_BODY, bb = (bo >> 8) < HT_MAXNB ? (int)(bo >> 8) : IDLE_BODY;
			const float4 La = S.ang4[ba], Lb = S.ang4[bb];
			float w = ab.z * La.x; w = __fmaf_rn(ab.w, La.y, w); w = __fmaf_rn(bt.x, La.z, w);
			w = __fmaf_rn(bt.y, Lb.x, w); w = __fmaf_rn(bt.z, Lb.y, w); w = __fmaf_rn(bt.w, Lb.z, w);
			float x = ((post ? sv.y : sv.x) - w) * gt.x;
			const float lo = sv.z - gt.y, hi = sv.w - gt.y;
			float imp = 0.0f;
			const int nrows = na - 32 * Q;
			auto cw16 = [](int nr) -> int { return (nr > 4 ? 2 : 0) | (nr > 8 ? 4 : 0) | (nr > 12 ? 8 : 0); };
			const int cwa0 = __builtin_amdgcn_readfirstlane(cw16(nrows)), cwa1 = __builtin_amdgcn_readfirstlane(cw16(nrows - 16));
#define BLK_ACASE(QQ) case QQ: if (nrows >= 16) blk_resolve16<QQ, 0, false>(x, lo, hi, imp, GA, 0); else blk_resolve16<QQ, 0, true>(x, lo, hi, imp, GA, cwa0); \
	if (nrows >= 32) blk_resolve16<QQ, 1, false>(x, lo, hi, imp, GA, 0); else if (nrows > 16) blk_resolve16<QQ, 1, true>(x, lo, hi, imp, GA, cwa1); break;
			switch (Q) { BLK_ACASE(0) BLK_ACASE(1) BLK_ACASE(2) default: BLK_ACASE(3) }
#undef BLK_ACASE
			if (act) R[AR_TORQUE] = gt.y + imp;
			const unsigned e = Q == 0 ? emA0 : Q == 1 ? emA1 : Q == 2 ? emA2 : emA3;
			const int src = (int)(e & 63);
			const float cf = (e & BLK_E_VALID) ? ((e & BLK_E_SIDE) ? 1.0f : -1.0f) : 0.0f;
			const float tx = gt.z * imp, ty = gt.w * imp, tz = ab.x * imp;
			float vx = blk_pull(src, tx) * cf, vy = blk_pull(src, ty) * cf, vz = blk_pull(src, tz) * cf;
			const blk_scan_mul sm = blk_scan_multipliers(e);
			blk_seg_scan3(vx, vy, vz, sm);
			if (e & BLK_E_TAIL)
			{
				const int body = (int)(e >> 16);
				float4 L = S.ang4[body];
				L.x += vx; L.y += vy; L.z += vz;
				S.ang4[body] = L;
			}
			__builtin_amdgcn_wave_barrier();
		}
	};
	for (int sweep = 0; sweep < total_sweeps; sweep++)
	{
		const bool post = sweep >= ph.iterations;
		const int tsoff = post ? 1 : 0;
		if (chain4)
		{
			if (c4_nblk > 0)
			{
				const int jq = (lane >> 2) & 3;
				if (idx_lds && g_lds) quad_blocks_run(scr, S.cidx, S.cg, S.csum, c4_e0, c4_nblk, c, jq, tsoff, lin_w, ang_w, c4_head, S.cextra, S.ccnt);
				else if (idx_lds) quad_blocks_run(scr, S.cidx, gG, S.csum, c4_e0, c4_nblk, c, jq, tsoff, lin_w, ang_w, c4_head, S.cextra, S.ccnt);
				else if (sums_lds) quad_blocks_run(scr, gidx, gG, S.csum, c4_e0, c4_nblk, c, jq, tsoff, lin_w, ang_w, c4_head, S.cextra, S.ccnt);
				else quad_blocks_run(scr, gidx, gG, gsum, c4_e0, c4_nblk, c, jq, tsoff, lin_w, ang_w, c4_head, S.cextra, S.ccnt);
			}
		}
		else
		{
			const int body = quad;
			const bool has = body < nb;
			const int cnt = has ? S.ccnt[body] : 0, start = has ? S.cstart[body] : 0;
			const int ex = has ? S.cextra[body] : -1;
			const int kswitch = ex >= 0 ? (cnt + 7) & ~7 : -1;
			const int total = ex >= 0 ? kswitch + S.ccnt[ex] : cnt;
			if (total > 0)
			{
				const float l = lin_w[4 * body + c], av = ang_w[4 * body + c];
				quad_body qb = { l, av };
				if (idx_lds) quad_chain_run(qb, scr, S.cidx + start, S.csum + start, total, c, tsoff, kswitch, lin_w, ang_w, body, ex);
				else if (sums_lds) quad_chain_run(qb, scr, gidx + start, S.csum + start, total, c, tsoff, kswitch, lin_w, ang_w, body, ex);
				else quad_chain_run(qb, scr, gidx + start, gsum + start, total, c, tsoff, kswitch, lin_w, ang_w, body, ex);
				const int last = ex >= 0 ? ex : body;
				if (c < 3) { lin_w[4 * last + c] = qb.l; ang_w[4 * last + c] = qb.av; }
			}
		}
		__builtin_amdgcn_wave_barrier();
		if (stats) { const long long t = clock64(); cyc_chain += t - t_mark; t_mark = t; }
		if (blocked) { if (!HT_DBG(a.dbg, 2)) { if (pool_lds) blocked_linear(S.pool, post); else blocked_linear(gpool, post); } }
		else if (!HT_DBG(a.dbg, 2) && nlev_lin > 0)
		{
			if (post) { if (pool_lds) linear_phase(S.pool, ht_true{}); else linear_phase(gpool, ht_true{}); }
			else { if (pool_lds) linear_phase(S.pool, ht_false{}); else linear_phase(gpool, ht_false{}); }
		}
		__builtin_amdgcn_wave_barrier();
		if (stats) { const long long t = clock64(); cyc_lin += t - t_mark; t_mark = t; }
		if (blocked) { if (!HT_DBG(a.dbg, 4)) { if (arec_lds) blocked_angular(S.arec, post); else blocked_angular(garec, post); } }
		else if (!HT_DBG(a.dbg, 4) && nlev_ang > 0)
		{
			if (post) { if (arec_lds) angular_phase(S.arec, ht_true{}); else angular_phase(garec, ht_true{}); }
			else { if (arec_lds) angular_phase(S.arec, ht_false{}); else angular_phase(garec, ht_false{}); }
		}
		__syncthreads();
		if (stats) { const long long t = clock64(); cyc_ang += t - t_mark; t_mark = t; }
		if (sweep + 1 == ph.iterations && lane < nb) calc_next_pose();
	}

	if (stats && lane == 0)
	{
		float *o = scr + (size_t)(a.scratch_stride - 1) * CREC;
		int mc = 0; for (int k = 0; k < nb; k++) if (S.ccnt[k] > mc) mc = S.ccnt[k];
		o[0] += 1.0f; o[1] += (float)cyc_chain; o[2] += (float)cyc_lin; o[3] += (float)cyc_ang; o[4] += (float)(clock64() - t_begin);
		o[5] += blocked ? (float)(t_c1 - t_c0) : (float)nlev_lin; o[6] += blocked ? (float)(t_c2 - t_c1) : (float)nlev_ang;       o[7] += (float)mc; o[8] += (float)n1; o[9] += (float)n2; o[10] += (float)na; o[11] += (float)(t_begin - t_entry);
		o[12] += (float)(t_m1 - t_entry); o[13] += (float)(t_m2 - t_m1); o[14] += (float)(t_m2b - t_m2); o[15] += (float)(t_m3 - t_m2b);
		if (HT_DBG(a.dbg, 262144)) { o[12] += (float)(t_l1 - t_m3) - (float)(t_m1 - t_entry); o[13] += (float)(t_l2 - t_l1) - (float)(t_m2 - t_m1); o[14] += (float)(t_l3 - t_l2) - (float)(t_m2b - t_m2); o[15] += (float)(t_l4 - t_l3) - (float)(t_m3 - t_m2b); }
		if (HT_DBG(a.dbg, 32768)) { o[12] += (float)cyc_bh - (float)(t_m1 - t_entry); o[13] += (float)cyc_br - (float)(t_m2 - t_m1); o[14] += (float)cyc_bg - (float)(t_m2b - t_m2); }
	}
	}
	if (lane < nb)
	{
		float *s = st + lane * HT_STATE_STRIDE;
		const float *bc = M.bodyc + lane * HT_BC;
		v3 pos = pos_next; v4 q = q_next;
		v3 lin = F3(S.lin4[lane]), ang = F3(S.ang4[lane]);
		const bool bad = isnan(lin.x) || isnan(lin.y) || isnan(lin.z) || isnan(pos.x) || isnan(pos.y) || isnan(pos.z) || isnan(ang.x) || isnan(ang.y) || isnan(ang.z)
		              || isnan(q.x) || isnan(q.y) || isnan(q.z) || isnan(q.w);
		if (bad) { pos = L3(bc + HT_BC_POS0); q = L4(bc + HT_BC_Q0); lin = V3(0, 0, 0); ang = V3(0, 0, 0); }
		if (a.zero_momenta) { lin = V3(0, 0, 0); ang = V3(0, 0, 0); }
		s[0] = pos.x; s[1] = pos.y; s[2] = pos.z; s[3] = q.x; s[4] = q.y; s[5] = q.z; s[6] = q.w;
		s[7] = lin.x; s[8] = lin.y; s[9] = lin.z; s[10] = ang.x; s[11] = ang.y; s[12] = ang.z;
		if (a.out_poses)
		{
			const v3 pu = apply(XF(pos, q), -L3(bc + HT_BC_COM));
			float *o = a.out_poses + ((size_t)b * nb + lane) * HT_POSE;
			o[0] = pu.x; o[1] = pu.y; o[2] = pu.z; o[3] = q.x; o[4] = q.y; o[5] = q.z; o[6] = q.w;
			if (lane == 0 && a.out_npts[b] < a.out_min_point_num) a.out_initializing[b] = 50;
		}
	}
	if (a.cost_out && lane == 0) a.cost_out[b] = (int)((clock64() - t_cost) >> 4);
}

__global__ __launch_bounds__(1024) void k_rank_desc(const int *__restrict__ work, int *__restrict__ order, int Ball, int stride, unsigned slots)
{
	__shared__ int rk_w[4096];
	if (!((slots >> blockIdx.x) & 1u)) return;
	const int f0 = blockIdx.y * 4096, B = Ball - f0 < 4096 ? Ball - f0 : 4096, B4 = (B + 3) & ~3;
	const int *w = work + (size_t)blockIdx.x * stride + f0;
	int *o = order + (size_t)blockIdx.x * stride + f0;
	for (int i = threadIdx.x; i < B4; i += 1024) rk_w[i] = i < B ? w[i] : -1;
	__syncthreads();
	for (int i = threadIdx.x; i < B; i += 1024)
	{
		const int wi = rk_w[i];
		int rank = 0;
		for (int j = 0; j < B4; j += 4)
		{
			const int4 k = *reinterpret_cast<const int4 *>(rk_w + j);
			rank += ((k.x > wi || (k.x == wi && j < i)) ? 1 : 0) + ((k.y > wi || (k.y == wi && j + 1 < i)) ? 1 : 0) + ((k.z > wi || (k.z == wi && j + 2 < i)) ? 1 : 0) + ((k.w > wi || (k.w == wi && j + 3 < i)) ? 1 : 0);
		}
		o[rank] = f0 + i;
	}
}
void ht_launch_rank_desc(const int *work, int *order, int B, int stride, unsigned slots, int nslots, hipStream_t s)
{
	hipLaunchKernelGGL(k_rank_desc, dim3(nslots, (B + 4095) / 4096), dim3(1024), 0, s, work, order, B, stride, slots);
}

#define SOLVE_ONLY_NCG 1440
static_assert(sizeof(lds_t<66, 1024, 126, 1024, 2, SOLVE_ONLY_NCG>) <= 40960, "the build for 1024 frames must fit four times into a CU's LDS");
static_assert(sizeof(lds_t<34, 584, 84, 0>) <= 20480, "the small build must leave room for eight frames per CU (160 KB of LDS)");
static_assert(HT_SCRATCH_TAIL * HT_CREC >= MAXG_CAP * LGRP + (MAXA_CAP_OF(4) + 4) * AROW + HT_CREC, "the tail of a frame's scratch slot must hold its linear groups, its angular records and the tuning record");
void ht_launch_solve(const ht_model_dev &M, const ht_physics_dev &ph, const solve_args &a, int B, hipStream_t s)
{
	const int pts = M.pts_bound > 0 ? M.pts_bound : M.pts_cap;
	const bool tile = M.nj + 8 + 1 <= 38 && pts <= 1024;
	int build = a.force_build;
	if (build == 7) { solve_args b = a; b.force_build = 0; b.two_body_levels = 1; ht_launch_solve(M, ph, b, B, s); return; }
	if (!build) build = tile ? (B <= 1024 && !a.shared_gpu ? 2 : 1) : 3;
	if (build >= 1 && build <= 3 && 13 + 6 * M.nj + a.ang_extra_bound > MAXA_CAP_OF(2)) build = 6;
	if (build == 2) hipLaunchKernelGGL((k_solve<66, 1024, 126, 1024, false, 2, SOLVE_ONLY_NCG>), dim3(B), dim3(64), 0, s, M, ph, a);
	else if (build == 1) hipLaunchKernelGGL((k_solve<34, 584, 84, 0>), dim3(B), dim3(64), 0, s, M, ph, a);
	else if (build == 3) hipLaunchKernelGGL((k_solve<71, 1520, 126, 1520>), dim3(B), dim3(64), 0, s, M, ph, a);
	else if (build == 5) hipLaunchKernelGGL((k_solve<71, 1520, 126, 1520, true, 4>), dim3(B), dim3(64), 0, s, M, ph, a);
	else if (build == 6) hipLaunchKernelGGL((k_solve<71, 1520, 126, 1520, false, 4>), dim3(B), dim3(64), 0, s, M, ph, a);
	else hipLaunchKernelGGL((k_solve<2, 64, 4, 0>), dim3(B), dim3(64), 0, s, M, ph, a);
}
```

hand_tracking_samples_amd/csrc/ht_solver_api.hip:

```cpp
#include <string.h>
#include <stdlib.h>
#include "ht_device.hpp"
#include "ht_host.hpp"
#include "ht_launch.hpp"

#define HIPCHK(ctx, call) do { hipError_t e_ = (call); if (e_ != hipSuccess) { (ctx)->err = std::string(#call) + ": " + hipGetErrorString(e_); return HT_ERR_HIP; } } while (0)
#define CHECK_READY(ctx) if (!(ctx)) return HT_ERR_ARG; if (!(ctx)->ready) { (ctx)->err = "context not initialised (ht_create failed)"; return HT_ERR_STATE; } ht_device_guard dev_guard_((ctx)->device)
#define CHECK_MODEL(ctx) do { if ((ctx)->cnn_only) { (ctx)->err = "this context was created without a hand model (CNN only)"; return HT_ERR_STATE; } } while (0)
#define CHECK_BATCH(ctx, B) do { if ((B) < 1 || (B) > (ctx)->B) { (ctx)->err = "batch exceeds the capacity given to ht_create"; return HT_ERR_ARG; } } while (0)
#define CHECK_RANGE(ctx, first, n) do { if ((first) < 0 || (n) < 1 || (first) + (n) > (ctx)->B) { (ctx)->err = "slot range exceeds the capacity given to ht_create"; return HT_ERR_ARG; } } while (0)

static int scratch_stride(const ht_ctx *ctx) { return (int)ht_scratch_rows((size_t)ctx->model.pts_cap, (size_t)ctx->model.nb); }

static int dev_alloc_points(ht_ctx *ctx)
{
	void *a = nullptr, *b = nullptr;
	HIPCHK(ctx, hipMalloc(&a, (size_t)ctx->B * ctx->model.pts_cap * sizeof(float4))); ctx->allocs.push_back(a); ctx->d_ptsv = (float4 *)a;
	if (!ctx->d_nptsv) { HIPCHK(ctx, hipMalloc(&b, (size_t)ctx->B * sizeof(int))); ctx->allocs.push_back(b); ctx->d_nptsv = (int *)b; }
	return HT_OK;
}
static cloud_records cloud_rec(ht_ctx *ctx) { cloud_records r = { ctx->d_scratch, scratch_stride(ctx), ctx->d_rowbody, ctx->phys.deltaT }; return r; }
static bool exact_solver(const ht_ctx *ctx) { return ctx->solver_build == 5 || ctx->solver_build == 8; }
static const cloud_records *rec_or_rows(const ht_ctx *ctx, const cloud_records *cr) { return exact_solver(ctx) ? nullptr : cr; }
static void exact_args(ht_ctx *ctx, solve_args &a, bool cloud)
// ... 545 lines not shown
	if (!ctx->d_frame_cams_in) { void *a = nullptr; HIPCHK(ctx, hipMalloc(&a, (size_t)ctx->B * HT_CAM * sizeof(float))); ctx->allocs.push_back(a); ctx->d_frame_cams_in = (float *)a; }
	HIPCHK(ctx, hipMemcpyAsync(ctx->d_frames, depth, (size_t)B * npx * sizeof(uint16_t), hipMemcpyHostToDevice, s));
	HIPCHK(ctx, hipMemcpyAsync(ctx->d_frame_cams_in, cams, (size_t)B * HT_CAM * sizeof(float), hipMemcpyHostToDevice, s));
	const frame_src fs = { side, side, 0.0f, side };
	int r = run_update(ctx, ctx->d_frames, ctx->d_frame_cams_in, nullptr, B, ctx->d_poses_out, nullptr, s, &fs);
	if (r) return r;
	HIPCHK(ctx, hipMemcpyAsync(poses_out, ctx->d_poses_out, (size_t)B * nb * HT_POSE * sizeof(float), hipMemcpyDeviceToHost, s));
	if (cnn_out) HIPCHK(ctx, hipMemcpyAsync(cnn_out, ctx->d_cnn_out, (size_t)B * HT_CNN_OUT * sizeof(float), hipMemcpyDeviceToHost, s));
	HIPCHK(ctx, hipStreamSynchronize(s));
	HIPCHK(ctx, hipGetLastError());
	return HT_OK;
}

extern "C" int ht_update_cnn_model_sync(ht_ctx *ctx, const uint16_t *depth, const float *cams, int w, int h, float segment_scale, int B, int apply_to_handmodel,
                                        float *poses_out, int *accepted_out, float *cnn_out)
{
	CHECK_READY(ctx); CHECK_MODEL(ctx); CHECK_BATCH(ctx, B);
	if (!depth || !cams) return HT_ERR_ARG;
	const bool tile = (w == 64 && h == 64);
	if (!tile && !frames_args_ok(ctx, w, h)) return HT_ERR_ARG;
	hipStream_t s = ctx->stream;
	const int nb = ctx->model.nb;
	const size_t npx = (size_t)w * h;
	const uint16_t *d_in; const float *d_cin;
	if (tile)
	{
		HIPCHK(ctx, hipMemcpyAsync(ctx->d_depth, depth, (size_t)B * npx * sizeof(uint16_t), hipMemcpyHostToDevice, s));
		HIPCHK(ctx, hipMemcpyAsync(ctx->d_cams, cams, (size_t)B * HT_CAM * sizeof(float), hipMemcpyHostToDevice, s));
		d_in = ctx->d_depth; d_cin = ctx->d_cams;
	}
	else
	{
		if (ctx->frames_cap < (size_t)B * npx) { void *a = nullptr; HIPCHK(ctx, hipMalloc(&a, (size_t)ctx->B * npx * sizeof(uint16_t))); ctx->allocs.push_back(a); ctx->d_frames = (uint16_t *)a; ctx->frames_cap = (size_t)ctx->B * npx; }
		if (!ctx->d_frame_cams_in) { void *a = nullptr; HIPCHK(ctx, hipMalloc(&a, (size_t)ctx->B * HT_CAM * sizeof(float))); ctx->allocs.push_back(a); ctx->d_frame_cams_in = (float *)a; }
		HIPCHK(ctx, hipMemcpyAsync(ctx->d_frames, depth, (size_t)B * npx * sizeof(uint16_t), hipMemcpyHostToDevice, s));
		HIPCHK(ctx, hipMemcpyAsync(ctx->d_frame_cams_in, cams, (size_t)B * HT_CAM * sizeof(float), hipMemcpyHostToDevice, s));
		d_in = ctx->d_frames; d_cin = ctx->d_frame_cams_in;
	}
	const frame_src fs = { w, h, segment_scale, 0 };
	int r = run_update(ctx, d_in, d_cin, nullptr, B, ctx->d_poses_out, nullptr, s, tile ? nullptr : &fs, apply_to_handmodel ? UPD_KICKSTART : UPD_CNN_MODEL);
	if (r) return r;
	if (poses_out) HIPCHK(ctx, hipMemcpyAsync(poses_out, ctx->d_poses_out, (size_t)B * nb * HT_POSE * sizeof(float), hipMemcpyDeviceToHost, s));
	if (accepted_out) HIPCHK(ctx, hipMemcpyAsync(accepted_out, ctx->d_accepted, (size_t)B * sizeof(int), hipMemcpyDeviceToHost, s));
	if (cnn_out) HIPCHK(ctx, hipMemcpyAsync(cnn_out, ctx->d_cnn_out, (size_t)B * HT_CNN_OUT * sizeof(float), hipMemcpyDeviceToHost, s));
	HIPCHK(ctx, hipStreamSynchronize(s));
	HIPCHK(ctx, hipGetLastError());
	if (accepted_out) for (int b = 0; b < B; b++) accepted_out[b] = accepted_out[b] != 0;
	if (!tile) { int over = 0; HIPCHK(ctx, hipMemcpy(&over, ctx->d_overflow, sizeof(int), hipMemcpyDeviceToHost)); if (over) { ctx->err = "ht_update_cnn_model: frame(s) with more in-range points than the solver's capacity"; return HT_ERR_ARG; } }
	return HT_OK;
}
__global__ void k_job_collect(float *__restrict__ hand, const float *__restrict__ other, const int *__restrict__ accepted, float *__restrict__ prev_err, const float *__restrict__ job_prev_err, int *__restrict__ initializing, int nb, int n)
{
	const int i = blockIdx.x * blockDim.x + threadIdx.x;
	if (i >= n * nb) return;
	const int f = i / nb;
	if (accepted[f]) { float *s = hand + (size_t)i * HT_STATE_STRIDE; const float *o = other + (size_t)i * HT_STATE_STRIDE; for (int k = 0; k < 7; k++) s[k] = o[k]; }
	if (i == f * nb) { prev_err[f] = job_prev_err[f]; const int v = initializing[f] - 1; initializing[f] = v < 0 ? 0 : v; }
}
extern "C" int ht_update_passes_sync(ht_ctx *ctx, const uint16_t *depth, const float *cams, int w, int h, int B, float *poses_out)
{
	CHECK_READY(ctx); CHECK_MODEL(ctx); CHECK_BATCH(ctx, B);
	if (!depth || !cams || !poses_out) return HT_ERR_ARG;
	const bool tile = (w == 64 && h == 64);
	if (!tile && !frames_args_ok(ctx, w, h)) return HT_ERR_ARG;
	hipStream_t s = ctx->stream;
	const int nb = ctx->model.nb;
	const size_t npx = (size_t)w * h;
	const uint16_t *d_in; const float *d_cin;
	if (tile)
	{
		HIPCHK(ctx, hipMemcpyAsync(ctx->d_depth, depth, (size_t)B * npx * sizeof(uint16_t), hipMemcpyHostToDevice, s));
		HIPCHK(ctx, hipMemcpyAsync(ctx->d_cams, cams, (size_t)B * HT_CAM * sizeof(float), hipMemcpyHostToDevice, s));
		d_in = ctx->d_depth; d_cin = ctx->d_cams;
	}
	else
	{
		if (ctx->frames_cap < (size_t)B * npx) { void *a = nullptr; HIPCHK(ctx, hipMalloc(&a, (size_t)ctx->B * npx * sizeof(uint16_t))); ctx->allocs.push_back(a); ctx->d_frames = (uint16_t *)a; ctx->frames_cap = (size_t)ctx->B * npx; }
		if (!ctx->d_frame_cams_in) { void *a = nullptr; HIPCHK(ctx, hipMalloc(&a, (size_t)ctx->B * HT_CAM * sizeof(float))); ctx->allocs.push_back(a); ctx->d_frame_cams_in = (float *)a; }
		HIPCHK(ctx, hipMemcpyAsync(ctx->d_frames, depth, (size_t)B * npx * sizeof(uint16_t), hipMemcpyHostToDevice, s));
		HIPCHK(ctx, hipMemcpyAsync(ctx->d_frame_cams_in, cams, (size_t)B * HT_CAM * sizeof(float), hipMemcpyHostToDevice, s));
		d_in = ctx->d_frames; d_cin = ctx->d_frame_cams_in;
	}
	const frame_src fs = { w, h, 0.17f, 0 };
	int r = run_update(ctx, d_in, d_cin, nullptr, B, ctx->d_poses_out, nullptr, s, tile ? nullptr : &fs, UPD_PASSES);
	if (r) return r;
	HIPCHK(ctx, hipMemcpyAsync(poses_out, ctx->d_poses_out, (size_t)B * nb * HT_POSE * sizeof(float), hipMemcpyDeviceToHost, s));
	HIPCHK(ctx, hipStreamSynchronize(s));
	HIPCHK(ctx, hipGetLastError());
	if (!tile) { int over = 0; HIPCHK(ctx, hipMemcpy(&over, ctx->d_overflow, sizeof(int), hipMemcpyDeviceToHost)); if (over) { ctx->err = "ht_update_passes: frame(s) with more in-range points than the context's point capacity holds"; return HT_ERR_ARG; } }
	return HT_OK;
}
extern "C" int ht_job_start(ht_ctx *job, ht_ctx *main, const uint16_t *depth, const float *cams, int w, int h, float segment_scale, int B)
{
	CHECK_READY(job); CHECK_MODEL(job); CHECK_BATCH(job, B);
	if (!main || !depth || !cams || main == job || main->device != job->device || main->model.nb != job->model.nb || B > main->B) { job->err = "ht_job_start: the two contexts must be different ones of one device with the same model"; return HT_ERR_ARG; }
	if (job->job_pending) { job->err = "ht_job_start: a job is in flight on this context (ht_job_collect takes it over)"; return HT_ERR_STATE; }
	const bool tile = (w == 64 && h == 64);
	if (!tile && !frames_args_ok(job, w, h)) return HT_ERR_ARG;
	hipStream_t s = job->stream;
	const int nb = job->model.nb;
	const size_t npx = (size_t)w * h, in_bytes = (size_t)B * npx * sizeof(uint16_t), cam_bytes = (size_t)B * HT_CAM * sizeof(float);
	if (!job->ev_job) HIPCHK(job, hipEventCreateWithFlags(&job->ev_job, hipEventDisableTiming));
	if (job->h_job_cap < in_bytes + cam_bytes) { if (job->h_job_in) (void)hipHostFree(job->h_job_in); job->h_job_in = nullptr; HIPCHK(job, hipHostMalloc(&job->h_job_in, in_bytes + cam_bytes, hipHostMallocDefault)); job->h_job_cap = in_bytes + cam_bytes; }
	HIPCHK(job, hipStreamSynchronize(main->stream));
	memcpy(job->h_job_in, depth, in_bytes); memcpy((char *)job->h_job_in + in_bytes, cams, cam_bytes);
	const uint16_t *d_in; const float *d_cin;
	if (tile)
	{
		HIPCHK(job, hipMemcpyAsync(job->d_depth, job->h_job_in, in_bytes, hipMemcpyHostToDevice, s));
		HIPCHK(job, hipMemcpyAsync(job->d_cams, (char *)job->h_job_in + in_bytes, cam_bytes, hipMemcpyHostToDevice, s));
		d_in = job->d_depth; d_cin = job->d_cams;
	}
	else
	{
		if (job->frames_cap < (size_t)B * npx) { void *a = nullptr; HIPCHK(job, hipMalloc(&a, (size_t)job->B * npx * sizeof(uint16_t))); job->allocs.push_back(a); job->d_frames = (uint16_t *)a; job->frames_cap = (size_t)job->B * npx; }
		if (!job->d_frame_cams_in) { void *a = nullptr; HIPCHK(job, hipMalloc(&a, (size_t)job->B * HT_CAM * sizeof(float))); job->allocs.push_back(a); job->d_frame_cams_in = (float *)a; }
		HIPCHK(job, hipMemcpyAsync(job->d_frames, job->h_job_in, in_bytes, hipMemcpyHostToDevice, s));
		HIPCHK(job, hipMemcpyAsync(job->d_frame_cams_in, (char *)job->h_job_in + in_bytes, cam_bytes, hipMemcpyHostToDevice, s));
		d_in = job->d_frames; d_cin = job->d_frame_cams_in;
	}
	HIPCHK(job, hipMemcpyAsync(job->d_state[0], main->d_state[0], (size_t)B * nb * HT_STATE_STRIDE * sizeof(float), hipMemcpyDeviceToDevice, s));
	ht_launch_set_pose(job->d_state[1], main->d_state[0], nb, B, 2, s);
	HIPCHK(job, hipMemcpyAsync(job->d_prev_err, main->d_prev_err, (size_t)B * sizeof(float), hipMemcpyDeviceToDevice, s));
	HIPCHK(job, hipMemcpyAsync(job->d_initializing, main->d_initializing, (size_t)B * sizeof(int), hipMemcpyDeviceToDevice, s));
	if (!job->ev_seed) HIPCHK(job, hipEventCreateWithFlags(&job->ev_seed, hipEventDisableTiming));
	HIPCHK(job, hipEventRecord(job->ev_seed, s));
	HIPCHK(job, hipStreamWaitEvent(main->stream, job->ev_seed, 0));
	const frame_src fs = { w, h, segment_scale, 0 };
	int r = run_update(job, d_in, d_cin, nullptr, B, job->d_poses_out, nullptr, s, tile ? nullptr : &fs, UPD_CNN_MODEL);
	if (r) { (void)hipStreamSynchronize(s); return r; }
	HIPCHK(job, hipEventRecord(job->ev_job, s));
	job->job_pending = true;
	return HT_OK;
}
extern "C" int ht_job_poll(ht_ctx *job, int *ready)
{
	if (!job || !ready) return HT_ERR_ARG;
	ht_device_guard dev_guard_(job->device);
	*ready = 0;
	if (!job->job_pending) return HT_OK;
	const hipError_t e = hipEventQuery(job->ev_job);
	if (e == hipSuccess) *ready = 1;
	else if (e != hipErrorNotReady) { job->err = std::string("ht_job_poll: ") + hipGetErrorString(e); return HT_ERR_HIP; }
	return HT_OK;
}
extern "C" int ht_job_wait(ht_ctx *job)
{
	if (!job) return HT_ERR_ARG;
	ht_device_guard dev_guard_(job->device);
	if (job->job_pending) HIPCHK(job, hipEventSynchronize(job->ev_job));
	return HT_OK;
}
extern "C" int ht_job_collect(ht_ctx *job, ht_ctx *main, int B, int *accepted_out)
{
	CHECK_READY(job); CHECK_MODEL(job); CHECK_BATCH(job, B);
	if (!main || main == job || main->device != job->device || main->model.nb != job->model.nb || B > main->B) return HT_ERR_ARG;
	if (!job->job_pending) { job->err = "ht_job_collect: no job in flight"; return HT_ERR_STATE; }
	HIPCHK(job, hipEventSynchronize(job->ev_job));
	const int nb = job->model.nb;
	hipLaunchKernelGGL(k_job_collect, dim3((B * nb + 255) / 256), dim3(256), 0, main->stream, main->d_state[0], job->d_state[1], job->d_accepted, main->d_prev_err, job->d_prev_err, main->d_initializing, nb, B);
	if (accepted_out) { HIPCHK(job, hipMemcpyAsync(accepted_out, job->d_accepted, (size_t)B * sizeof(int), hipMemcpyDeviceToHost, main->stream)); }
	HIPCHK(job, hipStreamSynchronize(main->stream));
	if (accepted_out) for (int b = 0; b < B; b++) accepted_out[b] = accepted_out[b] != 0;
	job->job_pending = false;
	return HT_OK;
}
extern "C" int ht_get_cnn_results(ht_ctx *ctx, int first, int n, float *cnn_input, float *cnn_output, float *analysis)
{
	CHECK_READY(ctx); CHECK_MODEL(ctx); CHECK_RANGE(ctx, first, n);
	HIPCHK(ctx, ht_sync_all(ctx));
	if (cnn_input) HIPCHK(ctx, hipMemcpy(cnn_input, ctx->d_cnn_in + (size_t)first * HT_CNN_IN, (size_t)n * HT_CNN_IN * sizeof(float), hipMemcpyDeviceToHost));
	if (cnn_output) HIPCHK(ctx, hipMemcpy(cnn_output, ctx->d_cnn_out + (size_t)first * HT_CNN_OUT, (size_t)n * HT_CNN_OUT * sizeof(float), hipMemcpyDeviceToHost));
	if (analysis) HIPCHK(ctx, hipMemcpy(analysis, ctx->d_analysis + (size_t)first * HT_ANALYSIS, (size_t)n * HT_ANALYSIS * sizeof(float), hipMemcpyDeviceToHost));
	return HT_OK;
}

extern "C" int ht_get_cnn_layers(ht_ctx *ctx, int first, int n, float *act1, float *act2, float *act3, float *logits)
{
	CHECK_READY(ctx); CHECK_RANGE(ctx, first, n);
	HIPCHK(ctx, ht_sync_all(ctx));
	if (act1) HIPCHK(ctx, hipMemcpy(act1, ctx->d_act1 + (size_t)first * 3600, (size_t)n * 3600 * sizeof(float), hipMemcpyDeviceToHost));
	if (act2) HIPCHK(ctx, hipMemcpy(act2, ctx->d_act2 + (size_t)first * 2304, (size_t)n * 2304 * sizeof(float), hipMemcpyDeviceToHost));
	if (act3)
	{
		std::vector<float> packed((size_t)n * 2048);
		HIPCHK(ctx, hipMemcpy(packed.data(), ctx->d_act3 + (size_t)first * 2048, (size_t)n * 2048 * sizeof(float), hipMemcpyDeviceToHost));
		for (int r = 0; r < n; r++) for (int c = 0; c < 2048; c++) act3[(size_t)r * 2048 + c] = packed[(size_t)r * 2048 + ((c & ~15) | ((c & 3) << 2) | ((c >> 2) & 3))];
	}
	if (logits) HIPCHK(ctx, hipMemcpy(logits, ctx->d_logits + (size_t)first * HT_CNN_OUT, (size_t)n * HT_CNN_OUT * sizeof(float), hipMemcpyDeviceToHost));
	return HT_OK;
}

extern "C" int ht_stage_fit_error(ht_ctx *ctx, int which, int B, float *err)
{
	CHECK_READY(ctx); CHECK_MODEL(ctx); CHECK_BATCH(ctx, B);
	if (!err || which < 0 || which > 1) return HT_ERR_ARG;
	hipStream_t s = ctx->stream;
	ht_launch_fit_error(ctx->model, ctx->d_state[which], ctx->d_pts, ctx->d_npts, ctx->d_depth, ctx->d_cams, 64, 64, ctx->par.bone_sum_error_scale, ctx->d_err_old, B, s);
	HIPCHK(ctx, hipMemcpyAsync(err, ctx->d_err_old, (size_t)B * sizeof(float), hipMemcpyDeviceToHost, s));
	HIPCHK(ctx, hipStreamSynchronize(s));
	HIPCHK(ctx, hipGetLastError());
	return HT_OK;
}
extern "C" int ht_stage_cloud_rows(ht_ctx *ctx, int which, int stride, int use_cam_origin, int B, float *rows, int *nrows)
{
	CHECK_READY(ctx); CHECK_MODEL(ctx); CHECK_BATCH(ctx, B);
	if (!rows || !nrows || which < 0 || which > 1 || stride < 1) return HT_ERR_ARG;
	hipStream_t s = ctx->stream;
	HIPCHK(ctx, hipMemsetAsync(ctx->d_rows, 0, (size_t)B * ctx->model.pts_cap * HT_ROW * sizeof(float), s));
	ht_launch_cloud_rows(ctx->model, ctx->d_state[which], ctx->d_pts, ctx->d_npts, ctx->d_cams, nullptr, stride, use_cam_origin, 0, ctx->par, ctx->d_rows, ctx->d_nrows, B, s);
	HIPCHK(ctx, hipMemcpy2DAsync(rows, HT_MAXPTS * HT_ROW * sizeof(float), ctx->d_rows, (size_t)ctx->model.pts_cap * HT_ROW * sizeof(float), HT_MAXPTS * HT_ROW * sizeof(float), B, hipMemcpyDeviceToHost, s));
	HIPCHK(ctx, hipMemcpyAsync(nrows, ctx->d_nrows, (size_t)B * sizeof(int), hipMemcpyDeviceToHost, s));
	HIPCHK(ctx, hipStreamSynchronize(s));
	HIPCHK(ctx, hipGetLastError());
	return HT_OK;
}
extern "C" int ht_stage_chamber(ht_ctx *ctx, int which, int B, float *rows, int *nrows)
{
	CHECK_READY(ctx); CHECK_MODEL(ctx); CHECK_BATCH(ctx, B);
	if (!rows || !nrows || which < 0 || which > 1) return HT_ERR_ARG;
	hipStream_t s = ctx->stream;
	const size_t per = (size_t)5 * ctx->model.nb * HT_ROW;
	HIPCHK(ctx, hipMemsetAsync(ctx->d_chamber, 0, (size_t)B * per * sizeof(float), s));
	ht_launch_chamber(ctx->model, ctx->d_state[which], ctx->d_pts, ctx->d_npts, ctx->par.min_point_num, ctx->par.boundary_planes, 10.0f, ctx->d_chamber, ctx->d_nchamber, B, s);
	HIPCHK(ctx, hipMemcpyAsync(rows, ctx->d_chamber, (size_t)B * per * sizeof(float), hipMemcpyDeviceToHost, s));
	HIPCHK(ctx, hipMemcpyAsync(nrows, ctx->d_nchamber, (size_t)B * sizeof(int), hipMemcpyDeviceToHost, s));
	HIPCHK(ctx, hipStreamSynchronize(s));
	HIPCHK(ctx, hipGetLastError());
	return HT_OK;
}
extern "C" int ht_stage_contacts(ht_ctx *ctx, int which, int B, int cap, float *contacts, int *ncontacts)
{
	CHECK_READY(ctx); CHECK_MODEL(ctx); CHECK_BATCH(ctx, B);
	if (!contacts || !ncontacts || which < 0 || which > 1 || cap < 1) return HT_ERR_ARG;
	hipStream_t s = ctx->stream;
	ht_launch_contacts(ctx->model, ctx->d_state[which], ctx->phys.driftmax, ctx->phys.jiggle_sin, nullptr, ctx->d_epa_ws, ctx->d_contacts, ctx->d_ncontacts, B, s, false, ctx->contact_kernel);
	std::vector<float> tmp((size_t)B * HT_MAXCONTACT * HT_CONTACT);
	HIPCHK(ctx, hipMemcpyAsync(tmp.data(), ctx->d_contacts, tmp.size() * sizeof(float), hipMemcpyDeviceToHost, s));
	HIPCHK(ctx, hipMemcpyAsync(ncontacts, ctx->d_ncontacts, (size_t)B * sizeof(int), hipMemcpyDeviceToHost, s));
	HIPCHK(ctx, hipStreamSynchronize(s));
	HIPCHK(ctx, hipGetLastError());
	const int ncopy = cap < HT_MAXCONTACT ? cap : HT_MAXCONTACT;
	for (int b = 0; b < B; b++) memcpy(contacts + (size_t)b * cap * HT_CONTACT, tmp.data() + (size_t)b * HT_MAXCONTACT * HT_CONTACT, (size_t)ncopy * HT_CONTACT * sizeof(float));
	return HT_OK;
}
extern "C" int ht_stage_fit(ht_ctx *ctx, int B)
{
	CHECK_READY(ctx); CHECK_MODEL(ctx); CHECK_BATCH(ctx, B);
	main_pass(ctx, B, ctx->stream);
	HIPCHK(ctx, hipStreamSynchronize(ctx->stream));
	HIPCHK(ctx, hipGetLastError());
	return HT_OK;
}
extern "C" int ht_stage_multistep(ht_ctx *ctx, const float *analysis, int B)
{
	CHECK_READY(ctx); CHECK_MODEL(ctx); CHECK_BATCH(ctx, B);
	if (!analysis) return HT_ERR_ARG;
	hipStream_t s = ctx->stream;
	HIPCHK(ctx, hipMemcpyAsync(ctx->d_analysis, analysis, (size_t)B * HT_ANALYSIS * sizeof(float), hipMemcpyHostToDevice, s));
	multistep(ctx, B, s);
	HIPCHK(ctx, hipStreamSynchronize(s));
	HIPCHK(ctx, hipGetLastError());
	return HT_OK;
}
extern "C" int ht_stage_multistep_range(ht_ctx *ctx, const float *analysis, int B, int from_step, int to_step)
{
	CHECK_READY(ctx); CHECK_MODEL(ctx); CHECK_BATCH(ctx, B);
	if (!analysis || from_step < 0 || to_step < from_step) return HT_ERR_ARG;
	hipStream_t s = ctx->stream;
	HIPCHK(ctx, hipMemcpyAsync(ctx->d_analysis, analysis, (size_t)B * HT_ANALYSIS * sizeof(float), hipMemcpyHostToDevice, s));
	multistep(ctx, B, s, from_step, to_step);
	HIPCHK(ctx, hipStreamSynchronize(s));
	HIPCHK(ctx, hipGetLastError());
	return HT_OK;
}
extern "C" int ht_stage_scratch_unibody(ht_ctx *ctx, const float *analysis, int B, int n_unibody)
{
	CHECK_READY(ctx); CHECK_MODEL(ctx); CHECK_BATCH(ctx, B);
	if (!analysis) return HT_ERR_ARG;
	hipStream_t s = ctx->stream;
	HIPCHK(ctx, hipMemcpyAsync(ctx->d_analysis, analysis, (size_t)B * HT_ANALYSIS * sizeof(float), hipMemcpyHostToDevice, s));
	reset_path(ctx, false, n_unibody, B, s, s);
	HIPCHK(ctx, hipStreamSynchronize(s));
	HIPCHK(ctx, hipGetLastError());
	return HT_OK;
}

extern "C" int ht_debug_solve_stats(ht_ctx *ctx, int B, float *out, int reset)
{
	if (!ctx || !ctx->ready || B < 1 || B > ctx->B) return HT_ERR_ARG;
	ht_device_guard dev_guard_(ctx->device);
	const int stride = scratch_stride(ctx);
	if (ht_sync_all(ctx) != hipSuccess) return HT_ERR_HIP;
	for (int b = 0; b < B; b++)
	{
		float *src = ctx->d_scratch + ((size_t)b * stride + (stride - 1)) * HT_CREC;
		if (out && hipMemcpy(out + (size_t)b * 16, src, 16 * sizeof(float), hipMemcpyDeviceToHost) != hipSuccess) return HT_ERR_HIP;
		if (reset && hipMemset(src, 0, 16 * sizeof(float)) != hipSuccess) return HT_ERR_HIP;
	}
	return HT_OK;
}
extern "C" int ht_debug_solver_build(ht_ctx *ctx, int which)
{
	if (!ctx || which < 0 || which > 8) return HT_ERR_ARG;
	if ((which == 5 || which == 8) && !ctx->d_exact_lin)
	{
		ht_device_guard dev_guard_(ctx->device);
		void *a = nullptr, *b = nullptr;
		HIPCHK(ctx, hipMalloc(&a, (size_t)ctx->B * HT_EX_LIN * HT_ROW * sizeof(float))); ctx->allocs.push_back(a); ctx->d_exact_lin = (float *)a;
		HIPCHK(ctx, hipMalloc(&b, (size_t)ctx->B * 256 * 8 * sizeof(float))); ctx->allocs.push_back(b); ctx->d_exact_ang = (float *)b;
	}
	ctx->solver_build = which;
	return HT_OK;
}
extern "C" int ht_debug_reset_organisation(ht_ctx *ctx, int *many)
{
	if (!ctx || !many) return HT_ERR_ARG;
	*many = ctx->last_reset_many;
	return HT_OK;
}
extern "C" int ht_debug_reset_flags(ht_ctx *ctx, int *flags, int n)
{
	if (!ctx || !flags || n < 0 || n > ctx->B) return HT_ERR_ARG;
	ht_device_guard dev_guard_(ctx->device);
	HIPCHK(ctx, hipStreamSynchronize(ctx->stream));
	HIPCHK(ctx, hipMemcpy(flags, ctx->d_flags, (size_t)n * sizeof(int), hipMemcpyDeviceToHost));
	return HT_OK;
}
extern "C" int ht_debug_contact_kernel(ht_ctx *ctx, int which)
{
	if (!ctx || which < 0 || which > 2) return HT_ERR_ARG;
	ctx->contact_kernel = which;
	return HT_OK;
}
extern "C" int ht_debug_solve_tables(ht_ctx *ctx, int on)
{
	if (!ctx || !ctx->ready) return HT_ERR_ARG;
	ht_device_guard dev_guard_(ctx->device);
	if (on < 0 || on > 2) return HT_ERR_ARG;
	if (on) { const int r = ht_alloc_solve_tables(ctx); if (r) return r; }
	ctx->solve_tables = on;
	return HT_OK;
}
extern "C" int ht_debug_solve_tables_header(ht_ctx *ctx, int B, int *hdr)
{
	if (!ctx || !ctx->ready || !hdr || B < 1 || B > ctx->B || !ctx->d_tables) return HT_ERR_ARG;
	ht_device_guard dev_guard_(ctx->device);
	if (ht_sync_all(ctx) != hipSuccess) return HT_ERR_HIP;
	if (hipMemcpy2D(hdr, 32 * sizeof(int), ctx->d_tables, (size_t)TB_WORDS * sizeof(float), 32 * sizeof(int), B, hipMemcpyDeviceToHost) != hipSuccess) return HT_ERR_HIP;
	return HT_OK;
}
extern "C" int ht_debug_contact_stats(ht_ctx *ctx, int B, float *out, int reset)
{
	if (!ctx || !ctx->ready || B < 1 || B > ctx->B) return HT_ERR_ARG;
	ht_device_guard dev_guard_(ctx->device);
	if (hipDeviceSynchronize() != hipSuccess) return HT_ERR_HIP;
	for (int b = 0; b < B; b++)
	{
		float *src = ctx->d_contacts + ((size_t)b * HT_MAXCONTACT + HT_MAXCONTACT - 2) * HT_CONTACT;
		if (out && hipMemcpy(out + (size_t)b * 24, src, 24 * sizeof(float), hipMemcpyDeviceToHost) != hipSuccess) return HT_ERR_HIP;
		if (reset && hipMemset(src, 0, 24 * sizeof(float)) != hipSuccess) return HT_ERR_HIP;
	}
	return HT_OK;
}

extern "C" int ht_segment_vr_dev(ht_ctx *ctx, const uint16_t *d_depth, const float *d_cams, int w, int h, int B, int entry_options, float wrange_lo, float wrange_hi, float diam,
                                 uint16_t *d_tiles, float *d_cams_out, void *stream)
{
	CHECK_READY(ctx);
	(void)wrange_lo;
	if (!d_depth || !d_cams || !d_tiles || !d_cams_out || B < 1) return HT_ERR_ARG;
	hipStream_t s = ht_user_stream(ctx, stream);
	if (w == 64 && h == 64)
	{
		HIPCHK(ctx, hipMemcpyAsync(d_tiles, d_depth, (size_t)B * 4096 * sizeof(uint16_t), hipMemcpyDeviceToDevice, s));
		HIPCHK(ctx, hipMemcpyAsync(d_cams_out, d_cams, (size_t)B * HT_CAM * sizeof(float), hipMemcpyDeviceToDevice, s));
		return HT_OK;
	}
	if (!ht_segment_supported(w, h)) { ctx->err = "ht_segment_vr: frame size must be a multiple of 4 and at most 320x240 pixels"; return HT_ERR_ARG; }
	ht_launch_segment(d_depth, d_cams, w, h, entry_options, wrange_hi, diam, d_tiles, d_cams_out, B, s);
	HIPCHK(ctx, hipGetLastError());
	return HT_OK;
}
extern "C" int ht_segment_vr(ht_ctx *ctx, const uint16_t *depth, const float *cams, int w, int h, int B, int entry_options, float wrange_lo, float wrange_hi, float diam,
                             uint16_t *tiles, float *cams_out)
{
	CHECK_READY(ctx);
	if (!depth || !cams || !tiles || !cams_out || B < 1 || w < 1 || h < 1) return HT_ERR_ARG;
	uint16_t *d_in = nullptr, *d_tiles = nullptr; float *d_cams = nullptr, *d_co = nullptr;
	const size_t nin = (size_t)B * w * h;
	int rc = HT_OK;
	if (hipMalloc((void **)&d_in, nin * sizeof(uint16_t)) != hipSuccess || hipMalloc((void **)&d_tiles, (size_t)B * 4096 * sizeof(uint16_t)) != hipSuccess ||
	    hipMalloc((void **)&d_cams, (size_t)B * HT_CAM * sizeof(float)) != hipSuccess || hipMalloc((void **)&d_co, (size_t)B * HT_CAM * sizeof(float)) != hipSuccess)
	{ ctx->err = "ht_segment_vr: out of device memory"; rc = HT_ERR_HIP; }
	hipStream_t s = ctx->stream;
	if (rc == HT_OK && (hipMemcpyAsync(d_in, depth, nin * sizeof(uint16_t), hipMemcpyHostToDevice, s) != hipSuccess ||
	                    hipMemcpyAsync(d_cams, cams, (size_t)B * HT_CAM * sizeof(float), hipMemcpyHostToDevice, s) != hipSuccess)) { ctx->err = "ht_segment_vr: upload failed"; rc = HT_ERR_HIP; }
	if (rc == HT_OK) rc = ht_segment_vr_dev(ctx, d_in, d_cams, w, h, B, entry_options, wrange_lo, wrange_hi, diam, d_tiles, d_co, s);
	if (rc == HT_OK && (hipMemcpyAsync(tiles, d_tiles, (size_t)B * 4096 * sizeof(uint16_t), hipMemcpyDeviceToHost, s) != hipSuccess ||
	                    hipMemcpyAsync(cams_out, d_co, (size_t)B * HT_CAM * sizeof(float), hipMemcpyDeviceToHost, s) != hipSuccess ||
	                    hipStreamSynchronize(s) != hipSuccess)) { ctx->err = "ht_segment_vr: download failed"; rc = HT_ERR_HIP; }
	(void)hipFree(d_in); (void)hipFree(d_tiles); (void)hipFree(d_cams); (void)hipFree(d_co);
	return rc;
}

static void drop_alloc(ht_ctx *ctx, void *o) { if (!o) return; for (auto &q : ctx->allocs) if (q == o) { q = ctx->allocs.back(); ctx->allocs.pop_back(); break; } (void)hipFree(o); }
static int user_rows_reserve(ht_ctx *ctx, int lin_cap, int ang_cap)
{
	if (lin_cap > ctx->user_lin_cap)
	{
		HIPCHK(ctx, ht_sync_all(ctx));
		void *a = nullptr, *b = nullptr;
		HIPCHK(ctx, hipMalloc(&a, (size_t)ctx->B * lin_cap * HT_ROW * sizeof(float)));
		if (hipMalloc(&b, (size_t)ctx->B * lin_cap * sizeof(unsigned short)) != hipSuccess) { (void)hipFree(a); ctx->err = "caller-built rows: out of device memory"; return HT_ERR_HIP; }
		drop_alloc(ctx, ctx->d_user_lin); drop_alloc(ctx, ctx->d_user_pos);
		ctx->allocs.push_back(a); ctx->d_user_lin = (float *)a; ctx->allocs.push_back(b); ctx->d_user_pos = (unsigned short *)b;
		ctx->user_lin_cap = lin_cap;
	}
	if (ang_cap > ctx->user_ang_cap)
	{
		HIPCHK(ctx, ht_sync_all(ctx));
		void *a = nullptr;
		HIPCHK(ctx, hipMalloc(&a, (size_t)ctx->B * ang_cap * HT_AROW * sizeof(float)));
		drop_alloc(ctx, ctx->d_user_ang);
		ctx->allocs.push_back(a); ctx->d_user_ang = (float *)a;
		ctx->user_ang_cap = ang_cap;
	}
	if (!ctx->d_user_n) { void *a = nullptr; HIPCHK(ctx, hipMalloc(&a, (size_t)4 * ctx->B * sizeof(int))); ctx->allocs.push_back(a); ctx->d_user_n = (int *)a; }
	return HT_OK;
}
static int upload_angulars(ht_ctx *ctx, int B, const float *angulars, int acap, const int *nangulars, std::vector<int> &na)
{
	na.assign(B, 0);
	for (int b = 0; b < B; b++)
	{
		na[b] = (angulars && nangulars) ? nangulars[b] : 0;
		if (na[b] < 0 || na[b] > acap || na[b] > 126 || 13 + 6 * ctx->model.nj + na[b] > 252) { ctx->err = "caller-built angular rows: a count is negative, exceeds the stride, exceeds 126 or leaves no room for the model's own rows among the 252 angular rows a solve keeps"; return HT_ERR_ARG; }
		for (int i = 0; i < na[b]; i++) { const float *r = angulars + ((size_t)b * acap + i) * HT_AROW; if ((int)r[0] >= ctx->model.nb || (int)r[1] >= ctx->model.nb) { ctx->err = "caller-built angular rows: body index out of range"; return HT_ERR_ARG; } }
	}
	if (acap > 0 && angulars) HIPCHK(ctx, hipMemcpy2D(ctx->d_user_ang, (size_t)ctx->user_ang_cap * HT_AROW * sizeof(float), angulars, (size_t)acap * HT_AROW * sizeof(float), (size_t)acap * HT_AROW * sizeof(float), B, hipMemcpyHostToDevice));
	HIPCHK(ctx, hipMemcpy(ctx->d_user_n + 3 * (size_t)ctx->B, na.data(), (size_t)B * sizeof(int), hipMemcpyHostToDevice));
	return HT_OK;
}
extern "C" int ht_fit_rows(ht_ctx *ctx, int which, int B, const float *points, int pcap, const int *npoints, const float *linears, int lcap, const int *nlinears,
                           const float *angulars, int acap, const int *nangulars, float microforce)
{
	CHECK_READY(ctx); CHECK_MODEL(ctx); CHECK_BATCH(ctx, B);
	if (which < 0 || which > 1 || pcap < 0 || lcap < 0 || acap < 0) return HT_ERR_ARG;
	const int nb = ctx->model.nb;
	std::vector<int> nl(B, 0), na;
	for (int b = 0; b < B; b++)
	{
		nl[b] = (linears && nlinears) ? nlinears[b] : 0;
		if (nl[b] < 0 || nl[b] > lcap || nl[b] > 5 * nb + 128) { ctx->err = "ht_fit_rows: a linear row count is negative, exceeds the stride or exceeds the 5 * bodies + 128 caller rows a frame's scratch slot holds"; return HT_ERR_ARG; }
		for (int i = 0; i < nl[b]; i++)
		{
			const float *r = linears + ((size_t)b * lcap + i) * HT_ROW;
			if ((int)r[0] >= 0 || (int)r[1] < 0 || (int)r[1] >= nb || r[15] != 0.0f) { ctx->err = "ht_fit_rows: the caller's linear rows must act on one body from the world (rb0 == NULL, no friction master); use ht_physics_update for general rows"; return HT_ERR_ARG; }
		}
	}
	{ const int r = user_rows_reserve(ctx, lcap > 1 ? lcap : 1, acap > 1 ? acap : 1); if (r) return r; }
	{ const int r = upload_angulars(ctx, B, angulars, acap, nangulars, na); if (r) return r; }
	{
		static const float none[3] = { 0, 0, 0 }; std::vector<int> zero(B, 0);
		const int r = (points && npoints && pcap > 0) ? ht_set_points(ctx, B, points, pcap, npoints) : ht_set_points(ctx, 1, none, 1, zero.data());
		if (r) return r;
		if (!(points && npoints && pcap > 0)) HIPCHK(ctx, hipMemset(ctx->d_npts, 0, (size_t)B * sizeof(int)));
	}
	if (lcap > 0 && linears) HIPCHK(ctx, hipMemcpy2D(ctx->d_user_lin, (size_t)ctx->user_lin_cap * HT_ROW * sizeof(float), linears, (size_t)lcap * HT_ROW * sizeof(float), (size_t)lcap * HT_ROW * sizeof(float), B, hipMemcpyHostToDevice));
	HIPCHK(ctx, hipMemcpy(ctx->d_user_n, nl.data(), (size_t)B * sizeof(int), hipMemcpyHostToDevice));
	hipStream_t s = ctx->stream;
	const bool coll = ctx->phys.use_collision != 0;
	ht_params par = ctx->par; par.microforce = microforce;
	const cloud_records cr = cloud_rec(ctx);
	ht_launch_cloud_rows(ctx->model, ctx->d_state[which], ctx->d_pts, ctx->d_npts, ctx->d_cams, nullptr, 1, 0, 1, par, ctx->d_rows, ctx->d_nrows, B, s, 0.0f, 0.0f, &cr);
	if (coll) ht_launch_contacts(ctx->model, ctx->d_state[which], ctx->phys.driftmax, ctx->phys.jiggle_sin, nullptr, ctx->d_epa_ws, ctx->d_contacts, ctx->d_ncontacts, B, s, false, ctx->contact_kernel);
	solve_args a;
	memset(&a, 0, sizeof a);
	a.sf_select = -1;
	a.caps = reinterpret_cast<int *>(ctx->d_epa_ws) + 2;
	a.rows_pre = ctx->d_user_lin; a.n_pre = ctx->d_user_n; a.pre_stride = ctx->user_lin_cap;
	a.cloud_body = ctx->d_rowbody; a.n_cloud = ctx->d_nrows;
	a.contacts = coll ? ctx->d_contacts : nullptr; a.ncontacts = ctx->d_ncontacts;
	a.ang_user = ctx->d_user_ang; a.n_ang_user = ctx->d_user_n + 3 * (size_t)ctx->B; a.ang_user_stride = ctx->user_ang_cap;
	{ int mx = 0; for (int v : na) mx = v > mx ? v : mx; a.ang_extra_bound = mx; }
	a.analysis = ctx->d_analysis; a.cams = ctx->d_cams;
	a.state = ctx->d_state[which]; a.scratch = ctx->d_scratch; a.scratch_stride = scratch_stride(ctx); a.batch = ctx->B;
	if (exact_solver(ctx)) { ctx->err = "the exact-order instantiation (ht_debug_solver_build 5) serves the update entry points only"; return HT_ERR_STATE; }
	a.force_build = ctx->solver_build;
	ctx->model.pts_bound = 0;
	ht_launch_solve(ctx->model, ctx->phys, a, B, s);
	HIPCHK(ctx, hipStreamSynchronize(s));
	HIPCHK(ctx, hipGetLastError());
	return HT_OK;
}
extern "C" int ht_physics_update(ht_ctx *ctx, int which, int B, const float *linears, int lcap, const int *nlinears, const float *angulars, int acap, const int *nangulars)
{
	CHECK_READY(ctx); CHECK_MODEL(ctx); CHECK_BATCH(ctx, B);
	if (which < 0 || which > 1 || lcap < 0 || acap < 0) return HT_ERR_ARG;
	const int nb = ctx->model.nb;
	std::vector<int> npre(B, 0), ntail(B, 0), ngrp(B, 0), na;
	std::vector<unsigned short> pos((size_t)B * (lcap > 1 ? lcap : 1), 0);
	int most_pre = 0;
	for (int b = 0; b < B; b++)
	{
		const int n = (linears && nlinears) ? nlinears[b] : 0;
		if (n < 0 || n > lcap) { ctx->err = "ht_physics_update: a linear row count is negative or exceeds the stride"; return HT_ERR_ARG; }
		const float *rows = linears + (size_t)b * lcap * HT_ROW;
		for (int i = 0; i < n; i++) if ((int)rows[i * HT_ROW] >= nb || (int)rows[i * HT_ROW + 1] >= nb || ((int)rows[i * HT_ROW] < 0 && (int)rows[i * HT_ROW + 1] < 0)) { ctx->err = "ht_physics_update: body index out of range"; return HT_ERR_ARG; }
		int p = 0;
		while (p < n && (int)rows[p * HT_ROW] < 0 && rows[p * HT_ROW + 15] == 0.0f && !(p + 1 < n && rows[(p + 1) * HT_ROW + 15] != 0.0f)) p++;
		npre[b] = p; ntail[b] = n - p; if (p > most_pre) most_pre = p;
		int g = -1, slot = 3, g0 = 0; int pa = -2, pb = -2;
		for (int i = p; i < n; i++)
		{
			const float *r = rows + (size_t)i * HT_ROW;
			const int fm = (int)r[15], ra = (int)r[0], rb = (int)r[1];
			const bool next_is_friction = i + 1 < n && rows[(size_t)(i + 1) * HT_ROW + 15] != 0.0f && fm == 0;
			if (fm != 0)
			{
				if (g < 0 || -fm != slot || slot > 2 || ra != pa || rb != pb) { ctx->err = "ht_physics_update: a friction row must directly follow its master row (friction_master -1, then -2) on the same bodies"; return HT_ERR_ARG; }
				for (int k = g0; k <= i; k++) pos[(size_t)b * lcap + (k - p)] |= 0x8000;
			}
			else if (g < 0 || slot > 2 || ra != pa || rb != pb || next_is_friction || (pos[(size_t)b * lcap + (g0 - p)] & 0x8000)) { g++; slot = 0; g0 = i; pa = ra; pb = rb; }
			pos[(size_t)b * lcap + (i - p)] |= (unsigned short)((g << 2) | slot);
			slot++;
		}
		ngrp[b] = g + 1;
		if (ngrp[b] > HT_MAXNJ) { ctx->err = "ht_physics_update: more than 32 groups of two-body rows in a frame"; return HT_ERR_ARG; }
	}
	if (most_pre > ctx->model.pts_cap) { const int r = ht_reserve_points_locked(ctx, most_pre); if (r) return r; }
	{ const int r = user_rows_reserve(ctx, lcap > 1 ? lcap : 1, acap > 1 ? acap : 1); if (r) return r; }
	{ const int r = upload_angulars(ctx, B, angulars, acap, nangulars, na); if (r) return r; }
	const size_t pc = (size_t)ctx->model.pts_cap;
	for (int b = 0; b < B; b++)
	{
		const float *rows = linears ? linears + (size_t)b * lcap * HT_ROW : nullptr;
		if (npre[b]) HIPCHK(ctx, hipMemcpy(ctx->d_rows + (size_t)b * pc * HT_ROW, rows, (size_t)npre[b] * HT_ROW * sizeof(float), hipMemcpyHostToDevice));
		if (ntail[b])
		{
			HIPCHK(ctx, hipMemcpy(ctx->d_user_lin + (size_t)b * ctx->user_lin_cap * HT_ROW, rows + (size_t)npre[b] * HT_ROW, (size_t)ntail[b] * HT_ROW * sizeof(float), hipMemcpyHostToDevice));
			HIPCHK(ctx, hipMemcpy(ctx->d_user_pos + (size_t)b * ctx->user_lin_cap, pos.data() + (size_t)b * lcap, (size_t)ntail[b] * sizeof(unsigned short), hipMemcpyHostToDevice));
		}
	}
	HIPCHK(ctx, hipMemcpy(ctx->d_nrows, npre.data(), (size_t)B * sizeof(int), hipMemcpyHostToDevice));
	HIPCHK(ctx, hipMemcpy(ctx->d_user_n + (size_t)ctx->B, ntail.data(), (size_t)B * sizeof(int), hipMemcpyHostToDevice));
	HIPCHK(ctx, hipMemcpy(ctx->d_user_n + 2 * (size_t)ctx->B, ngrp.data(), (size_t)B * sizeof(int), hipMemcpyHostToDevice));
	hipStream_t s = ctx->stream;
	const bool coll = ctx->phys.use_collision != 0;
	if (coll) ht_launch_contacts(ctx->model, ctx->d_state[which], ctx->phys.driftmax, ctx->phys.jiggle_sin, nullptr, ctx->d_epa_ws, ctx->d_contacts, ctx->d_ncontacts, B, s, false, ctx->contact_kernel);
	solve_args a;
	memset(&a, 0, sizeof a);
	a.sf_select = -1;
	a.caps = reinterpret_cast<int *>(ctx->d_epa_ws) + 2;
	a.rows_cloud = ctx->d_rows; a.n_cloud = ctx->d_nrows;
	a.contacts = coll ? ctx->d_contacts : nullptr; a.ncontacts = ctx->d_ncontacts;
	a.ang_user = ctx->d_user_ang; a.n_ang_user = ctx->d_user_n + 3 * (size_t)ctx->B; a.ang_user_stride = ctx->user_ang_cap;
	{ int mx = 0; for (int v : na) mx = v > mx ? v : mx; a.ang_extra_bound = mx; }
	a.lin_tail = ctx->d_user_lin; a.n_lin_tail = ctx->d_user_n + (size_t)ctx->B; a.lin_tail_stride = ctx->user_lin_cap;
	a.lin_tail_pos = ctx->d_user_pos; a.n_tail_groups = ctx->d_user_n + 2 * (size_t)ctx->B;
	a.no_model_rows = 1;
	a.analysis = ctx->d_analysis; a.cams = ctx->d_cams;
	a.state = ctx->d_state[which]; a.scratch = ctx->d_scratch; a.scratch_stride = scratch_stride(ctx); a.batch = ctx->B;
	if (exact_solver(ctx)) { ctx->err = "the exact-order instantiation (ht_debug_solver_build 5) serves the update entry points only"; return HT_ERR_STATE; }
	a.force_build = ctx->solver_build;
	ctx->model.pts_bound = 0;
	ht_launch_solve(ctx->model, ctx->phys, a, B, s);
	HIPCHK(ctx, hipStreamSynchronize(s));
	HIPCHK(ctx, hipGetLastError());
	return HT_OK;
}

extern "C" int ht_slowfit(ht_ctx *ctx, int B, int hold, const float *refpose, int steps, int select_rb, const float *spoint, const float *rbpoint, const float *crays, int ncray)
{
	CHECK_READY(ctx); CHECK_MODEL(ctx); CHECK_BATCH(ctx, B);
	const int nb = ctx->model.nb;
	if (steps < 1 || ncray < 0 || ncray > 8 || select_rb >= nb || (select_rb >= 0 && (!spoint || !rbpoint)) || (ncray > 0 && !crays)) { ctx->err = "ht_slowfit: bad arguments"; return HT_ERR_ARG; }
	hipStream_t s = ctx->stream;
	if (!ctx->d_sf_ref)
	{
		void *p = nullptr, *q = nullptr;
		HIPCHK(ctx, hipMalloc(&p, (size_t)ctx->B * nb * HT_POSE * sizeof(float))); ctx->allocs.push_back(p); ctx->d_sf_ref = (float *)p;
		HIPCHK(ctx, hipMalloc(&q, (size_t)ctx->B * 8 * 4 * sizeof(float))); ctx->allocs.push_back(q); ctx->d_sf_crays = (float *)q;
	}
	const bool rel = hold && refpose;
	if (rel) HIPCHK(ctx, hipMemcpyAsync(ctx->d_sf_ref, refpose, (size_t)B * nb * HT_POSE * sizeof(float), hipMemcpyHostToDevice, s));
	if (ncray) HIPCHK(ctx, hipMemcpyAsync(ctx->d_sf_crays, crays, (size_t)B * 8 * 4 * sizeof(float), hipMemcpyHostToDevice, s));
	const bool coll = ctx->phys.use_collision != 0;
	for (int st = 0; st < steps; st++)
	{
		const bool cloud = st < steps - 1;
		const cloud_records cr = cloud_rec(ctx);
		if (cloud) ht_launch_cloud_rows(ctx->model, ctx->d_state[0], ctx->d_pts, ctx->d_npts, ctx->d_cams, nullptr, 1, 0, 4, ctx->par, ctx->d_rows, ctx->d_nrows, B, s,
		                                1.0f * (float)(steps - st) / (float)steps, 0.1f * (float)(st < steps - 2), &cr);
		if (coll) ht_launch_contacts(ctx->model, ctx->d_state[0], ctx->phys.driftmax, ctx->phys.jiggle_sin, nullptr, ctx->d_epa_ws, ctx->d_contacts, ctx->d_ncontacts, B, s, false, ctx->contact_kernel);
		solve_args a;
		memset(&a, 0, sizeof a);
		a.caps = reinterpret_cast<int *>(ctx->d_epa_ws) + 2;
		a.cloud_body = cloud ? ctx->d_rowbody : nullptr; a.n_cloud = ctx->d_nrows;
		a.contacts = coll ? ctx->d_contacts : nullptr; a.ncontacts = ctx->d_ncontacts;
		a.analysis = ctx->d_analysis; a.cams = ctx->d_cams;
		a.state = ctx->d_state[0]; a.scratch = ctx->d_scratch; a.scratch_stride = scratch_stride(ctx); a.batch = ctx->B;
		a.sf_ncray = st < 5 ? ncray : 0; a.sf_crays = ctx->d_sf_crays; a.sf_select = select_rb;
		for (int i = 0; i < 3; i++) { a.sf_spoint[i] = spoint ? spoint[i] : 0.0f; a.sf_rbpoint[i] = rbpoint ? rbpoint[i] : 0.0f; }
		a.ray_rows = (a.sf_ncray > 0 || select_rb >= 0) ? 1 : 0;
		a.sf_refpose = rel ? ctx->d_sf_ref : nullptr; a.sf_hold = rel ? hold : 0;
		a.ang_extra_bound = rel ? 3 * ctx->model.nj : 0;
// ... 28 lines not shown
```

Measured before the change: 232,200 frames/s.

## Split solver block into two waves overlapping chain-list build with angular setup

The build-2 solve kernel now launches 128 threads per frame. A second wave builds the contact chain lists and coupling blocks while the first wave does the angular-row and level setup, and the results are handed over through a small LDS array. Intra-wave barriers replace block barriers where only one wave participates. This is meant to hide the serial chain-building latency, but it doubles the threads per block, which may reduce how many frames fit per CU and adds register pressure under the launch bounds.

After: 233,500 frames/s, median of 6. About the same (+0.6%).

```diff
diff --git a/hand_tracking_samples_amd/csrc/ht_launch.hpp b/hand_tracking_samples_amd/csrc/ht_launch.hpp
--- a/hand_tracking_samples_amd/csrc/ht_launch.hpp
+++ b/hand_tracking_samples_amd/csrc/ht_launch.hpp
@@ -22,6 +22,7 @@
 	int shared_gpu;
 	const int *frame_order; int *cost_out;
 	int two_body_levels;
+	int one_wave;
 	int force_build;
 	float *out_poses; const int *out_npts; int *out_initializing; int out_min_point_num;
 	int ang_extra_bound;
diff --git a/hand_tracking_samples_amd/csrc/ht_solver.hip b/hand_tracking_samples_amd/csrc/ht_solver.hip
--- a/hand_tracking_samples_amd/csrc/ht_solver.hip
+++ b/hand_tracking_samples_amd/csrc/ht_solver.hip
@@ -1,6 +1,6 @@
 #include "ht_solve_shared.hpp"
 
-template <int NGRP_, int NSUM_, int NANG_, int NIDX_, int AS_ = 2, int NCG_ = 0> struct lds_t
+template <int NGRP_, int NSUM_, int NANG_, int NIDX_, int AS_ = 2, int NCG_ = 0, int NX_ = 0> struct lds_t
 {
 	static constexpr int NGRP = NGRP_, NSUM = NSUM_, NANG = NANG_, NIDX = NIDX_, MAXA2 = MAXA2_OF(AS_), NCG = NCG_;
 	static constexpr int LIDLE = MAXG - 1;
@@ -11,6 +11,7 @@
 	float csum[NSUM];
 	unsigned short cidx[NIDX > 0 ? NIDX : 2];
 	float cg[NCG];
+	int c4x[NX_];
 	int ccnt[HT_MAXNB], cstart[HT_MAXNB];
 	signed char cextra[HT_MAXNB];
 	union
@@ -87,12 +88,17 @@
 }
 
 #define EX_LIN HT_EX_LIN
-template <int NGRP_, int NSUM_, int NANG_, int NIDX_, bool EXACT = false, int AS = 2, int NCG_ = 0>
-__global__ __launch_bounds__(64, 2) void k_solve(ht_model_dev M, ht_physics_dev ph, solve_args a)
+template <int NGRP_, int NSUM_, int NANG_, int NIDX_, bool EXACT = false, int AS = 2, int NCG_ = 0, int PW = 1>
+__global__ __launch_bounds__(64 * PW, 2) void k_solve(ht_model_dev M, ht_physics_dev ph, solve_args a)
 {
-	__shared__ lds_t<NGRP_, NSUM_, NANG_, NIDX_, AS, NCG_> S;
+	static_assert(PW == 1 || !EXACT, "the exact-order instantiation keeps one wave");
+	__shared__ lds_t<NGRP_, NSUM_, NANG_, NIDX_, AS, NCG_, (PW > 1 ? 13 : 0)> S;
 	constexpr int ASLOTS = AS, MAXA2 = MAXA2_OF(AS), MAXA_LDS = MAXA_CAP_OF(AS);
-	const int lane = threadIdx.x;
+	const int lane = PW > 1 ? (int)(threadIdx.x & 63) : (int)threadIdx.x;
+	const int wave = PW > 1 ? __builtin_amdgcn_readfirstlane((int)(threadIdx.x >> 6)) : 0;
+	const bool two = PW > 1 && blockDim.x > 64;
+	const int cw = two ? 1 : 0;
+	auto sync_own = [&]() { if constexpr (PW > 1) { __threadfence_block(); __builtin_amdgcn_wave_barrier(); } else __syncthreads(); };
 	const int b = a.frame_order ? a.frame_order[blockIdx.x] : (int)blockIdx.x;
 	if (a.active_flag && !a.active_flag[b]) return;
 	const long long t_cost = a.cost_out ? clock64() : 0;
@@ -121,7 +127,7 @@
 		}
 	}
 
-	if (lane < nb)
+	if (wave == 0 && lane < nb)
 	{
 		const float *s = st + lane * HT_STATE_STRIDE;
 		const float *bc = M.bodyc + lane * HT_BC;
@@ -136,11 +142,11 @@
 		m3 I = world_inertia(V4(s[3], s[4], s[5], s[6]), LM(bc + HT_BC_TINV), bc[HT_BC_MASSINV]);
 		S.I4[lane][0] = make_float4(I.x.x, I.x.y, I.x.z, 0.0f); S.I4[lane][1] = make_float4(I.y.x, I.y.y, I.y.z, 0.0f); S.I4[lane][2] = make_float4(I.z.x, I.z.y, I.z.z, 0.0f);
 	}
-	if (lane < nj && !fast_pose) for (int i = 0; i < 6; i++) S.jr[lane][i] = M.jointc[lane * HT_JC + HT_JC_RMIN + i];
-	if (lane == 0) S.nray = fast_chain && a.ray_rows ? t_npre : 0;
+	if (wave == 0 && lane < nj && !fast_pose) for (int i = 0; i < 6; i++) S.jr[lane][i] = M.jointc[lane * HT_JC + HT_JC_RMIN + i];
+	if (wave == 0 && lane == 0) S.nray = fast_chain && a.ray_rows ? t_npre : 0;
 	__syncthreads();
 
-	if (nb >= 17 && !a.no_model_rows && !fast_pose)
+	if (wave == 0 && nb >= 17 && !a.no_model_rows && !fast_pose)
 	{
 		if (lane < 4)
 		{
@@ -159,7 +165,7 @@
 			S.jr[kb - 1][4] = up ? r1 : 0.0f;
 		}
 	}
-	if (fast_chain) {}
+	if (fast_chain || wave != cw) {}
 	else if (a.ray_rows && a.sf_ncray + (a.sf_select >= 0) > 0 && lane == 8)
 	{
 		int k = 0;
@@ -227,6 +233,221 @@
 	__syncthreads();
 	if (HT_DBG(a.dbg, 256)) return;
 	const long long t_m1 = HT_DBG(a.dbg, 2048) ? clock64() : 0;
+	const int rec_cap = a.scratch_stride - HT_SCRATCH_TAIL;
+	float *scr = a.scratch + (size_t)b * a.scratch_stride * CREC;
+	const int npre_g = a.rows_pre ? a.n_pre[b] : 0;
+	const int npre = a.ray_rows ? S.nray : npre_g;
+	const int ncl = (a.rows_cloud || a.cloud_body) ? a.n_cloud[b] : 0;
+	const int n1 = npre + ncl;
+	const int pre_base = M.pts_cap, noop_idx = rec_cap - 1;
+	const int npad_max = 7 * (nb > 16 ? nb - 16 : 0);
+	const int nlist = n1 + (npad_max > 3 * nb ? npad_max : 3 * nb) + (QUAD_CHAIN_SLACK > QUAD_BLOCK_SLACK ? QUAD_CHAIN_SLACK : QUAD_BLOCK_SLACK);
+	const bool sums_lds = nlist <= S.NSUM;
+	const bool idx_lds = sums_lds && nlist <= S.NIDX && rec_cap <= 65536;
+	float *const gsum = a.scratch + (size_t)a.batch * a.scratch_stride * CREC + (size_t)b * a.scratch_stride;
+	unsigned *const gidx = reinterpret_cast<unsigned *>(a.scratch + (size_t)a.batch * a.scratch_stride * (CREC + 1)) + (size_t)b * a.scratch_stride;
+	float *const gG = a.scratch + (size_t)a.batch * a.scratch_stride * (CREC + 2) + (size_t)b * a.scratch_stride * 4;
+	const bool chain4 = !EXACT && !HT_DBG(a.dbg, 65536);
+	int c4_e0 = 0, c4_nblk = 0, c4_head = 0, c4_total = 0;
+	bool g_lds = false;
+	long long t_l1 = 0, t_l2 = 0, t_l3 = 0, t_l4 = 0;
+	auto pre_ptr = [&](int i) -> const float * { return a.ray_rows ? S.ray[i] : a.rows_pre + ((size_t)b * a.pre_stride + i) * HT_ROW; };
+	auto chain_lists = [&]() {
+		if (sums_lds) { for (int i = lane; i < nlist; i += 64) S.csum[i] = 0.0f; }
+		else for (int i = lane; i < nlist && i < a.scratch_stride; i += 64) gsum[i] = 0.0f;
+		if (fast_chain) { if (idx_lds) for (int i = lane; i < nlist; i += 64) S.cidx[i] = (unsigned short)gidx[i]; }
+		else if (idx_lds) { for (int i = lane; i < nlist; i += 64) S.cidx[i] = (unsigned short)noop_idx; }
+		else for (int i = lane; i < nlist && i < a.scratch_stride; i += 64) gidx[i] = (unsigned)noop_idx;
+		if (lane == 0 && !fast_chain) quad_write_noop(scr + (size_t)noop_idx * CREC);
+		auto body_of = [&](int i) -> int {
+			if (i < npre) return (int)pre_ptr(i)[1];
+			if (a.cloud_body) return (int)a.cloud_body[(size_t)b * M.pts_cap + (i - npre)];
+			return (int)a.rows_cloud[((size_t)b * M.pts_cap + (i - npre)) * HT_ROW + 1];
+		};
+		sync_own();
+		int mycnt = 0;
+		if (!fast_chain)
+		for (int base = 0; base < n1; base += 64)
+		{
+			const int i = base + lane;
+			int body = (i < n1) ? body_of(i) : -1;
+			unsigned long long todo = __ballot(body >= 0);
+			while (todo)
+			{
+				const int leader = __ffsll((long long)todo) - 1;
+				const int bb = __builtin_amdgcn_readlane(body, leader);
+				const unsigned long long m = __ballot(body == bb);
+				if (lane == bb) mycnt += __popcll(m);
+				todo &= ~m;
+			}
+		}
+		t_l1 = HT_DBG(a.dbg, 262144) ? clock64() : 0;
+		int c4_start = 0, c4_next = -1;
+		int myblk = (lane < nb && !HT_DBG(a.dbg, 1)) ? (mycnt + 3) >> 2 : 0;
+		if (fast_chain)
+		{
+			c4_e0 = t_e0; c4_nblk = t_nblk; c4_head = t_head; c4_total = t_total;
+			if (lane < HT_MAXNB) { myblk = reinterpret_cast<const int *>(T + TB_CCNT)[lane]; c4_next = reinterpret_cast<const int *>(T + TB_CNEXT)[lane]; }
+		}
+		else if (chain4)
+		{
+			int myrank = 0;
+			for (int k = 0; k < nb; k++) { const int o = __builtin_amdgcn_readlane(myblk, k); myrank += (o > myblk || (o == myblk && k < lane)) ? 1 : 0; }
+			if (lane < nb) S.cstart[myrank] = lane;
+			__builtin_amdgcn_fence(__ATOMIC_SEQ_CST, "wavefront");
+			__builtin_amdgcn_wave_barrier();
+			const int sorted = lane < nb ? S.cstart[lane] : 0;
+			int ld0 = 0, ld1 = 0, ld2 = 0, ld3 = 0, la0 = -1, la1 = -1, la2 = -1, la3 = -1, hd0 = 0, hd1 = 0, hd2 = 0, hd3 = 0, myrow = 0, mypos = 0;
+			for (int r = 0; r < nb; r++)
+			{
+				const int bb = __builtin_amdgcn_readlane(sorted, r);
+				const int blk = __builtin_amdgcn_readlane(myblk, bb);
+				if (blk == 0) break;
+				int row = 0, best = ld0;
+				if (ld1 < best) { row = 1; best = ld1; }
+				if (ld2 < best) { row = 2; best = ld2; }
+				if (ld3 < best) { row = 3; best = ld3; }
+				const int prev = row == 0 ? la0 : row == 1 ? la1 : row == 2 ? la2 : la3;
+				if (lane == bb) { myrow = row; mypos = best; }
+				if (lane == prev) c4_next = bb;
+				if (prev < 0) { if (row == 0) hd0 = bb; else if (row == 1) hd1 = bb; else if (row == 2) hd2 = bb; else hd3 = bb; }
+				if (row == 0) { la0 = bb; ld0 += blk; } else if (row == 1) { la1 = bb; ld1 += blk; } else if (row == 2) { la2 = bb; ld2 += blk; } else { la3 = bb; ld3 += blk; }
+			}
+			const int sg1 = 4 * ld0, sg2 = sg1 + 4 * ld1, sg3 = sg2 + 4 * ld2;
+			c4_total = ld0 + ld1 + ld2 + ld3;
+			c4_start = (myrow == 0 ? 0 : myrow == 1 ? sg1 : myrow == 2 ? sg2 : sg3) + 4 * mypos;
+			const int R = lane >> 4;
+			c4_e0 = R == 0 ? 0 : R == 1 ? sg1 : R == 2 ? sg2 : sg3; c4_nblk = R == 0 ? ld0 : R == 1 ? ld1 : R == 2 ? ld2 : ld3; c4_head = R == 0 ? hd0 : R == 1 ? hd1 : R == 2 ? hd2 : hd3;
+		}
+		int myextra = -1, myhost = -1;
+		if (!fast_chain)
+		{
+			int avail = (lane < 16 && lane < nb) ? mycnt : 0x7fffff;
+			for (int e = 16; e < nb; e++)
+			{
+				int key = (avail << 6) | lane;
+	#pragma unroll
+				for (int o = 1; o < 64; o <<= 1) { const int v = __shfl_xor(key, o); key = v < key ? v : key; }
+				const int h = key & 63;
+				if (lane == h) { myextra = e; avail = 0x7fffff; }
+				if (lane == e) myhost = h;
+			}
+		}
+		const int extracnt = __shfl(mycnt, myextra >= 0 ? myextra : lane);
+		const int mylen = lane >= 16 ? 0 : (myextra >= 0 && extracnt > 0 ? ((mycnt + 7) & ~7) + extracnt : mycnt);
+		if (myextra >= 0 && extracnt == 0) myextra = -1;
+		int mystart = mylen;
+	#pragma unroll
+		for (int o = 1; o < 64; o <<= 1) { int v = __shfl_up(mystart, o); if (lane >= o) mystart += v; }
+		mystart -= mylen;
+		{
+			const int hs = __shfl(mystart, myhost >= 0 ? myhost : lane), hc = __shfl(mycnt, myhost >= 0 ? myhost : lane);
+			if (myhost >= 0) mystart = hs + ((hc + 7) & ~7);
+		}
+		if (chain4) { mystart = c4_start; if (lane < HT_MAXNB) { S.ccnt[lane] = myblk; S.cstart[lane] = mystart; S.cextra[lane] = (signed char)c4_next; } }
+		else if (lane < HT_MAXNB) { S.ccnt[lane] = HT_DBG(a.dbg, 1) ? 0 : mycnt; S.cstart[lane] = mystart; S.cextra[lane] = (signed char)(HT_DBG(a.dbg, 1) ? -1 : myextra); }
+		int myrun = 0;
+		t_l2 = HT_DBG(a.dbg, 262144) ? clock64() : 0;
+		if (!fast_chain)
+		for (int base = 0; base < n1; base += 64)
+		{
+			const int i = base + lane;
+			int body = (i < n1) ? body_of(i) : -1;
+			int dst = -1;
+			unsigned long long todo = __ballot(body >= 0);
+			while (todo)
+			{
+				const int leader = __ffsll((long long)todo) - 1;
+				const int bb = __builtin_amdgcn_readlane(body, leader);
+				const unsigned long long m = __ballot(body == bb);
+				const int segbase = __builtin_amdgcn_readlane(mystart + myrun, bb);
+				if (body == bb) dst = segbase + __popcll(m & ((1ull << lane) - 1ull));
+				if (lane == bb) myrun += __popcll(m);
+				todo &= ~m;
+			}
+			if (body >= 0)
+			{
+				const bool made = i >= npre && a.cloud_body;
+				const int src = i < npre ? pre_base + i : i - npre;
+				if (src < noop_idx && dst < nlist - QUAD_CHAIN_SLACK)
+				{
+					if (idx_lds) S.cidx[dst] = (unsigned short)src; else if (dst < a.scratch_stride) gidx[dst] = (unsigned)src;
+					if (!made)
+					{
+						const float *r = i < npre ? pre_ptr(i) : a.rows_cloud + ((size_t)b * M.pts_cap + (i - npre)) * HT_ROW;
+						const v3 p1 = L3(r + 5), n = L3(r + 8);
+						const v3 r1 = qrot(L4(S.q[body]), p1);
+						const m3 Ib = body_I(S, body);
+						const float impulsed = S.lin4[body].w + dot(cross(mul(Ib, cross(r1, n)), r1), n);
+						const float ts = r[11] / dt;
+						quad_write_record(scr + (size_t)src * CREC, r1, n, Ib, S.lin4[body].w, ts, fmin_std(ts, r[12]), impulsed, r[13] * dt, r[14] * dt);
+					}
+				}
+			}
+		}
+		t_l3 = HT_DBG(a.dbg, 262144) ? clock64() : 0;
+	};
+	auto chain_couplings = [&]() {
+		g_lds = idx_lds && S.NCG > 0 && QUAD_G_BLOCK * (c4_total + 4) <= S.NCG;
+		if (fast_chain)
+		{
+			if (g_lds) { for (int i = lane; i < QUAD_G_BLOCK * c4_total; i += 64) S.cg[i] = gG[i]; __threadfence_block(); sync_own(); }
+		}
+		else if (chain4 && !HT_DBG(a.dbg, 131072))
+		{
+			const int quad_ = lane >> 2, c_ = lane & 3;
+			for (int blk0 = quad_; blk0 < c4_total; blk0 += 64)
+			{
+				float4 r_[4][4];
+	#pragma unroll
+				for (int u = 0; u < 4; u++)
+	#pragma unroll
+					for (int j = 0; j < 4; j++)
+					{
+						const int blk = blk0 + 16 * u, e = 4 * blk + j;
+						const unsigned x = (blk < c4_total) ? (idx_lds ? (unsigned)S.cidx[e] : gidx[e]) : (unsigned)noop_idx;
+						r_[u][j] = reinterpret_cast<const float4 *>(scr + (size_t)x * CREC)[c_];
+					}
+	#pragma unroll
+				for (int u = 0; u < 4; u++)
+				{
+					const int blk = blk0 + 16 * u;
+					auto coup = [&](int j, int i) -> float {
+						const float p = __fmaf_rn(r_[u][j].z, r_[u][i].y, r_[u][j].x * r_[u][i].w);
+						const float t = dpp<QP_PREV>(p) + p;
+						return -(dpp<QP_PREV>(t) + p);
+					};
+					const float g10 = coup(1, 0), g20 = coup(2, 0), g21 = coup(2, 1), g30 = coup(3, 0), g31 = coup(3, 1), g32 = coup(3, 2);
+					if (c_ == 2 && blk < c4_total && 4 * blk + 3 < a.scratch_stride)
+					{
+						float2 *o = reinterpret_cast<float2 *>((g_lds ? S.cg : gG) + QUAD_G_BLOCK * blk);
+						o[0] = make_float2(g30, g31); o[1] = make_float2(g32, g20); o[2] = make_float2(g21, 0.0f); o[3] = make_float2(g10, 0.0f); o[4] = make_float2(0.0f, 0.0f);
+					}
+				}
+			}
+			__threadfence_block();
+			sync_own();
+		}
+		t_l4 = HT_DBG(a.dbg, 262144) ? clock64() : 0;
+	};
+	if constexpr (PW > 1)
+	{
+		if (wave == cw)
+		{
+			chain_lists();
+			__threadfence_block();
+			sync_own();
+			chain_couplings();
+			if ((lane & 15) == 0) { S.c4x[lane >> 4] = c4_e0; S.c4x[4 + (lane >> 4)] = c4_nblk; S.c4x[8 + (lane >> 4)] = c4_head; }
+			if (lane == 0) S.c4x[12] = c4_total;
+		}
+		if (wave == 1)
+		{
+			__threadfence_block();
+			__syncthreads();
+			return;
+		}
+	}
 	const bool rel = a.sf_refpose && a.sf_hold;
 	const int na_user = a.ang_user ? (a.n_ang_user[b] < MAXA_LDS ? a.n_ang_user[b] : MAXA_LDS) : 0;
 	int na_pre, na;
@@ -247,7 +468,7 @@
 		if (lane <= nj) { S.rprefix[lane] = na_fix + rpre; S.aprefix[lane] = na_pre + apre; }
 		for (int k = 0; k < acnt; k++) if (na_pre + apre + k < MAXA2) S.rowj[na_pre + apre + k] = (unsigned char)lane;
 	}
-	__syncthreads();
+	sync_own();
 	if (na > MAXA_LDS && a.caps && lane == 0) atomicAdd(a.caps, 1);
 	if (na > MAXA2) na = MAXA2;
 	arow AR[ASLOTS];
@@ -338,8 +559,6 @@
 	const int nt = a.lin_tail ? a.n_lin_tail[b] : 0, ngt = a.lin_tail ? a.n_tail_groups[b] : 0;
 	const int n2 = nt + 3 * njg + 3 * nc, ng2 = ngt + njg + nc;
 	const bool seq_lin = ng2 > MAXG - 1;
-	const int rec_cap = a.scratch_stride - HT_SCRATCH_TAIL;
-	float *scr = a.scratch + (size_t)b * a.scratch_stride * CREC;
 	const bool pool_lds = ng2 + 1 <= S.NGRP;
 	float *const gpool = scr + (size_t)rec_cap * CREC, *const garec = gpool + MAXG_CAP * LGRP;
 	float *const pool = pool_lds ? S.pool : gpool;
@@ -347,7 +566,7 @@
 	{
 		for (int i = lane; i < ngt * LGRP; i += 64) pool[i] = ((i % LGRP) >= LG_RINV && (i % LGRP) < LG_RINV + 3) ? 1.0f : 0.0f;
 		__threadfence_block();
-		__syncthreads();
+		sync_own();
 	}
 	if (fast_pose)
 	{
@@ -441,7 +660,7 @@
 		S.lorder[S.LIDLE] = (unsigned)ng2 | ((unsigned)IDLE_BODY << 16) | ((unsigned)IDLE_BODY << 24);
 	}
 	__threadfence_block();
-	__syncthreads();
+	sync_own();
 	const long long t_m2b = HT_DBG(a.dbg, 2048) ? clock64() : 0;
 	if (na > MAXA_LDS) na = MAXA_LDS;
 	bool blocked = false;
@@ -465,7 +684,7 @@
 		if (head && k <= MAXA_RUNS) S.gst[k] = (unsigned char)r;
 		nga += __popcll(m);
 	}
-	__syncthreads();
+	sync_own();
 	if (nga > MAXA_RUNS)
 	{
 		if (a.caps && lane == 0) atomicAdd(a.caps, 1);
@@ -500,158 +719,12 @@
 			S.aorder[MAXA2] = (unsigned)na | (1u << 8) | ((unsigned)IDLE_BODY << 16) | ((unsigned)IDLE_BODY << 24);
 		}
 	}
-	__syncthreads();
+	sync_own();
 	const int nlev_lin = S.nlev_lin, nlev_ang = S.nlev_ang;
 	if (HT_DBG(a.dbg, 64)) return;
 	const long long t_m3 = HT_DBG(a.dbg, 2048) ? clock64() : 0;
 
-	const int npre_g = a.rows_pre ? a.n_pre[b] : 0;
-	const int npre = a.ray_rows ? S.nray : npre_g;
-	const int ncl = (a.rows_cloud || a.cloud_body) ? a.n_cloud[b] : 0;
-	const int n1 = npre + ncl;
-	const int pre_base = M.pts_cap, noop_idx = rec_cap - 1;
-	const int npad_max = 7 * (nb > 16 ? nb - 16 : 0);
-	const int nlist = n1 + (npad_max > 3 * nb ? npad_max : 3 * nb) + (QUAD_CHAIN_SLACK > QUAD_BLOCK_SLACK ? QUAD_CHAIN_SLACK : QUAD_BLOCK_SLACK);
-	const bool sums_lds = nlist <= S.NSUM;
-	const bool idx_lds = sums_lds && nlist <= S.NIDX && rec_cap <= 65536;
-	float *const gsum = a.scratch + (size_t)a.batch * a.scratch_stride * CREC + (size_t)b * a.scratch_stride;
-	unsigned *const gidx = reinterpret_cast<unsigned *>(a.scratch + (size_t)a.batch * a.scratch_stride * (CREC + 1)) + (size_t)b * a.scratch_stride;
-	float *const gG = a.scratch + (size_t)a.batch * a.scratch_stride * (CREC + 2) + (size_t)b * a.scratch_stride * 4;
-	if (sums_lds) { for (int i = lane; i < nlist; i += 64) S.csum[i] = 0.0f; }
-	else for (int i = lane; i < nlist && i < a.scratch_stride; i += 64) gsum[i] = 0.0f;
-	if (fast_chain) { if (idx_lds) for (int i = lane; i < nlist; i += 64) S.cidx[i] = (unsigned short)gidx[i]; }
-	else if (idx_lds) { for (int i = lane; i < nlist; i += 64) S.cidx[i] = (unsigned short)noop_idx; }
-	else for (int i = lane; i < nlist && i < a.scratch_stride; i += 64) gidx[i] = (unsigned)noop_idx;
-	if (lane == 0 && !fast_chain) quad_write_noop(scr + (size_t)noop_idx * CREC);
-	auto pre_ptr = [&](int i) -> const float * { return a.ray_rows ? S.ray[i] : a.rows_pre + ((size_t)b * a.pre_stride + i) * HT_ROW; };
-	auto body_of = [&](int i) -> int {
-		if (i < npre) return (int)pre_ptr(i)[1];
-		if (a.cloud_body) return (int)a.cloud_body[(size_t)b * M.pts_cap + (i - npre)];
-		return (int)a.rows_cloud[((size_t)b * M.pts_cap + (i - npre)) * HT_ROW + 1];
-	};
-	__syncthreads();
-	int mycnt = 0;
-	if (!fast_chain)
-	for (int base = 0; base < n1; base += 64)
-	{
-		const int i = base + lane;
-		int body = (i < n1) ? body_of(i) : -1;
-		unsigned long long todo = __ballot(body >= 0);
-		while (todo)
-		{
-			const int leader = __ffsll((long long)todo) - 1;
-			const int bb = __builtin_amdgcn_readlane(body, leader);
-			const unsigned long long m = __ballot(body == bb);
-			if (lane == bb) mycnt += __popcll(m);
-			todo &= ~m;
-		}
-	}
-	const long long t_l1 = HT_DBG(a.dbg, 262144) ? clock64() : 0;
-	const bool chain4 = !EXACT && !HT_DBG(a.dbg, 65536);
-	int c4_e0 = 0, c4_nblk = 0, c4_head = 0, c4_start = 0, c4_next = -1, c4_total = 0;
-	int myblk = (lane < nb && !HT_DBG(a.dbg, 1)) ? (mycnt + 3) >> 2 : 0;
-	if (fast_chain)
-	{
-		c4_e0 = t_e0; c4_nblk = t_nblk; c4_head = t_head; c4_total = t_total;
-		if (lane < HT_MAXNB) { myblk = reinterpret_cast<const int *>(T + TB_CCNT)[lane]; c4_next = reinterpret_cast<const int *>(T + TB_CNEXT)[lane]; }
-	}
-	else if (chain4)
-	{
-		int myrank = 0;
-		for (int k = 0; k < nb; k++) { const int o = __builtin_amdgcn_readlane(myblk, k); myrank += (o > myblk || (o == myblk && k < lane)) ? 1 : 0; }
-		if (lane < nb) S.cstart[myrank] = lane;
-		__builtin_amdgcn_fence(__ATOMIC_SEQ_CST, "wavefront");
-		__builtin_amdgcn_wave_barrier();
-		const int sorted = lane < nb ? S.cstart[lane] : 0;
-		int ld0 = 0, ld1 = 0, ld2 = 0, ld3 = 0, la0 = -1, la1 = -1, la2 = -1, la3 = -1, hd0 = 0, hd1 = 0, hd2 = 0, hd3 = 0, myrow = 0, mypos = 0;
-		for (int r = 0; r < nb; r++)
-		{
-			const int bb = __builtin_amdgcn_readlane(sorted, r);
-			const int blk = __builtin_amdgcn_readlane(myblk, bb);
-			if (blk == 0) break;
-			int row = 0, best = ld0;
-			if (ld1 < best) { row = 1; best = ld1; }
-			if (ld2 < best) { row = 2; best = ld2; }
-			if (ld3 < best) { row = 3; best = ld3; }
-			const int prev = row == 0 ? la0 : row == 1 ? la1 : row == 2 ? la2 : la3;
-			if (lane == bb) { myrow = row; mypos = best; }
-			if (lane == prev) c4_next = bb;
-			if (prev < 0) { if (row == 0) hd0 = bb; else if (row == 1) hd1 = bb; else if (row == 2) hd2 = bb; else hd3 = bb; }
-			if (row == 0) { la0 = bb; ld0 += blk; } else if (row == 1) { la1 = bb; ld1 += blk; } else if (row == 2) { la2 = bb; ld2 += blk; } else { la3 = bb; ld3 += blk; }
-		}
-		const int sg1 = 4 * ld0, sg2 = sg1 + 4 * ld1, sg3 = sg2 + 4 * ld2;
-		c4_total = ld0 + ld1 + ld2 + ld3;
-		c4_start = (myrow == 0 ? 0 : myrow == 1 ? sg1 : myrow == 2 ? sg2 : sg3) + 4 * mypos;
-		const int R = lane >> 4;
-		c4_e0 = R == 0 ? 0 : R == 1 ? sg1 : R == 2 ? sg2 : sg3; c4_nblk = R == 0 ? ld0 : R == 1 ? ld1 : R == 2 ? ld2 : ld3; c4_head = R == 0 ? hd0 : R == 1 ? hd1 : R == 2 ? hd2 : hd3;
-	}
-	int myextra = -1, myhost = -1;
-	if (!fast_chain)
-	{
-		int avail = (lane < 16 && lane < nb) ? mycnt : 0x7fffff;
-		for (int e = 16; e < nb; e++)
-		{
-			int key = (avail << 6) | lane;
-#pragma unroll
-			for (int o = 1; o < 64; o <<= 1) { const int v = __shfl_xor(key, o); key = v < key ? v : key; }
-			const int h = key & 63;
-			if (lane == h) { myextra = e; avail = 0x7fffff; }
-			if (lane == e) myhost = h;
-		}
-	}
-	const int extracnt = __shfl(mycnt, myextra >= 0 ? myextra : lane);
-	const int mylen = lane >= 16 ? 0 : (myextra >= 0 && extracnt > 0 ? ((mycnt + 7) & ~7) + extracnt : mycnt);
-	if (myextra >= 0 && extracnt == 0) myextra = -1;
-	int mystart = mylen;
-#pragma unroll
-	for (int o = 1; o < 64; o <<= 1) { int v = __shfl_up(mystart, o); if (lane >= o) mystart += v; }
-	mystart -= mylen;
-	{
-		const int hs = __shfl(mystart, myhost >= 0 ? myhost : lane), hc = __shfl(mycnt, myhost >= 0 ? myhost : lane);
-		if (myhost >= 0) mystart = hs + ((hc + 7) & ~7);
-	}
-	if (chain4) { mystart = c4_start; if (lane < HT_MAXNB) { S.ccnt[lane] = myblk; S.cstart[lane] = mystart; S.cextra[lane] = (signed char)c4_next; } }
-	else if (lane < HT_MAXNB) { S.ccnt[lane] = HT_DBG(a.dbg, 1) ? 0 : mycnt; S.cstart[lane] = mystart; S.cextra[lane] = (signed char)(HT_DBG(a.dbg, 1) ? -1 : myextra); }
-	int myrun = 0;
-	const long long t_l2 = HT_DBG(a.dbg, 262144) ? clock64() : 0;
-	if (!fast_chain)
-	for (int base = 0; base < n1; base += 64)
-	{
-		const int i = base + lane;
-		int body = (i < n1) ? body_of(i) : -1;
-		int dst = -1;
-		unsigned long long todo = __ballot(body >= 0);
-		while (todo)
-		{
-			const int leader = __ffsll((long long)todo) - 1;
-			const int bb = __builtin_amdgcn_readlane(body, leader);
-			const unsigned long long m = __ballot(body == bb);
-			const int segbase = __builtin_amdgcn_readlane(mystart + myrun, bb);
-			if (body == bb) dst = segbase + __popcll(m & ((1ull << lane) - 1ull));
-			if (lane == bb) myrun += __popcll(m);
-			todo &= ~m;
-		}
-		if (body >= 0)
-		{
-			const bool made = i >= npre && a.cloud_body;
-			const int src = i < npre ? pre_base + i : i - npre;
-			if (src < noop_idx && dst < nlist - QUAD_CHAIN_SLACK)
-			{
-				if (idx_lds) S.cidx[dst] = (unsigned short)src; else if (dst < a.scratch_stride) gidx[dst] = (unsigned)src;
-				if (!made)
-				{
-					const float *r = i < npre ? pre_ptr(i) : a.rows_cloud + ((size_t)b * M.pts_cap + (i - npre)) * HT_ROW;
-					const v3 p1 = L3(r + 5), n = L3(r + 8);
-					const v3 r1 = qrot(L4(S.q[body]), p1);
-					const m3 Ib = body_I(S, body);
-					const float impulsed = S.lin4[body].w + dot(cross(mul(Ib, cross(r1, n)), r1), n);
-					const float ts = r[11] / dt;
-					quad_write_record(scr + (size_t)src * CREC, r1, n, Ib, S.lin4[body].w, ts, fmin_std(ts, r[12]), impulsed, r[13] * dt, r[14] * dt);
-				}
-			}
-		}
-	}
-	const long long t_l3 = HT_DBG(a.dbg, 262144) ? clock64() : 0;
+	if constexpr (PW == 1) chain_lists();
 	v3 ABA0[ASLOTS], ABA1[ASLOTS];
 #pragma unroll
 	for (int s = 0; s < ASLOTS; s++)
@@ -663,47 +736,13 @@
 	}
 	__threadfence_block();
 	__syncthreads();
-	const bool g_lds = idx_lds && S.NCG > 0 && QUAD_G_BLOCK * (c4_total + 4) <= S.NCG;
-	if (fast_chain)
-	{
-		if (g_lds) { for (int i = lane; i < QUAD_G_BLOCK * c4_total; i += 64) S.cg[i] = gG[i]; __threadfence_block(); __syncthreads(); }
-	}
-	else if (chain4 && !HT_DBG(a.dbg, 131072))
-	{
-		const int quad_ = lane >> 2, c_ = lane & 3;
-		for (int blk0 = quad_; blk0 < c4_total; blk0 += 64)
-		{
-			float4 r_[4][4];
-#pragma unroll
-			for (int u = 0; u < 4; u++)
-#pragma unroll
-				for (int j = 0; j < 4; j++)
-				{
-					const int blk = blk0 + 16 * u, e = 4 * blk + j;
-					const unsigned x = (blk < c4_total) ? (idx_lds ? (unsigned)S.cidx[e] : gidx[e]) : (unsigned)noop_idx;
-					r_[u][j] = reinterpret_cast<const float4 *>(scr + (size_t)x * CREC)[c_];
-				}
-#pragma unroll
-			for (int u = 0; u < 4; u++)
-			{
-				const int blk = blk0 + 16 * u;
-				auto coup = [&](int j, int i) -> float {
-					const float p = __fmaf_rn(r_[u][j].z, r_[u][i].y, r_[u][j].x * r_[u][i].w);
-					const float t = dpp<QP_PREV>(p) + p;
-					return -(dpp<QP_PREV>(t) + p);
-				};
-				const float g10 = coup(1, 0), g20 = coup(2, 0), g21 = coup(2, 1), g30 = coup(3, 0), g31 = coup(3, 1), g32 = coup(3, 2);
-				if (c_ == 2 && blk < c4_total && 4 * blk + 3 < a.scratch_stride)
-				{
-					float2 *o = reinterpret_cast<float2 *>((g_lds ? S.cg : gG) + QUAD_G_BLOCK * blk);
-					o[0] = make_float2(g30, g31); o[1] = make_float2(g32, g20); o[2] = make_float2(g21, 0.0f); o[3] = make_float2(g10, 0.0f); o[4] = make_float2(0.0f, 0.0f);
-				}
-			}
-		}
-		__threadfence_block();
-		__syncthreads();
-	}
-	const long long t_l4 = HT_DBG(a.dbg, 262144) ? clock64() : 0;
+	if constexpr (PW == 1) chain_couplings();
+	else
+	{
+		const int R = lane >> 4;
+		c4_e0 = S.c4x[R]; c4_nblk = S.c4x[4 + R]; c4_head = S.c4x[8 + R]; c4_total = S.c4x[12];
+		g_lds = idx_lds && S.NCG > 0 && QUAD_G_BLOCK * (c4_total + 4) <= S.NCG;
+	}
 	v3 pos_next = V3(0, 0, 0); v4 q_next = V4(0, 0, 0, 1);
 	auto calc_next_pose = [&]() {
 		const float *bc = M.bodyc + lane * HT_BC;
@@ -1425,7 +1464,7 @@
 }
 
 #define SOLVE_ONLY_NCG 1440
-static_assert(sizeof(lds_t<66, 1024, 126, 1024, 2, SOLVE_ONLY_NCG>) <= 40960, "the build for 1024 frames must fit four times into a CU's LDS");
+static_assert(sizeof(lds_t<66, 1024, 126, 1024, 2, SOLVE_ONLY_NCG, 13>) <= 40960, "the build for 1024 frames must fit four times into a CU's LDS");
 static_assert(sizeof(lds_t<34, 584, 84, 0>) <= 20480, "the small build must leave room for eight frames per CU (160 KB of LDS)");
 static_assert(HT_SCRATCH_TAIL * HT_CREC >= MAXG_CAP * LGRP + (MAXA_CAP_OF(4) + 4) * AROW + HT_CREC, "the tail of a frame's scratch slot must hold its linear groups, its angular records and the tuning record");
 void ht_launch_solve(const ht_model_dev &M, const ht_physics_dev &ph, const solve_args &a, int B, hipStream_t s)
@@ -1434,9 +1473,10 @@
 	const bool tile = M.nj + 8 + 1 <= 38 && pts <= 1024;
 	int build = a.force_build;
 	if (build == 7) { solve_args b = a; b.force_build = 0; b.two_body_levels = 1; ht_launch_solve(M, ph, b, B, s); return; }
+	if (build == 9 || build == 10) { solve_args b = a; b.force_build = build == 10 ? 2 : 0; b.one_wave = 1; ht_launch_solve(M, ph, b, B, s); return; }
 	if (!build) build = tile ? (B <= 1024 && !a.shared_gpu ? 2 : 1) : 3;
 	if (build >= 1 && build <= 3 && 13 + 6 * M.nj + a.ang_extra_bound > MAXA_CAP_OF(2)) build = 6;
-	if (build == 2) hipLaunchKernelGGL((k_solve<66, 1024, 126, 1024, false, 2, SOLVE_ONLY_NCG>), dim3(B), dim3(64), 0, s, M, ph, a);
+	if (build == 2) hipLaunchKernelGGL((k_solve<66, 1024, 126, 1024, false, 2, SOLVE_ONLY_NCG, 2>), dim3(B), dim3(a.one_wave ? 64 : 128), 0, s, M, ph, a);
 	else if (build == 1) hipLaunchKernelGGL((k_solve<34, 584, 84, 0>), dim3(B), dim3(64), 0, s, M, ph, a);
 	else if (build == 3) hipLaunchKernelGGL((k_solve<71, 1520, 126, 1520>), dim3(B), dim3(64), 0, s, M, ph, a);
 	else if (build == 5) hipLaunchKernelGGL((k_solve<71, 1520, 126, 1520, true, 4>), dim3(B), dim3(64), 0, s, M, ph, a);
diff --git a/hand_tracking_samples_amd/csrc/ht_solver_api.hip b/hand_tracking_samples_amd/csrc/ht_solver_api.hip
--- a/hand_tracking_samples_amd/csrc/ht_solver_api.hip
+++ b/hand_tracking_samples_amd/csrc/ht_solver_api.hip
@@ -871,7 +871,7 @@
 }
 extern "C" int ht_debug_solver_build(ht_ctx *ctx, int which)
 {
-	if (!ctx || which < 0 || which > 8) return HT_ERR_ARG;
+	if (!ctx || which < 0 || which > 10) return HT_ERR_ARG;
 	if ((which == 5 || which == 8) && !ctx->d_exact_lin)
 	{
 		ht_device_guard dev_guard_(ctx->device);
```
